# stateless-consensus/phant

Measured on NVIDIA B200. Metric: mpt_proofs_verified_per_sec, higher is better.
Workload: dtype u64

## Files before the change

### phant_b200/csrc/abi.cu

```cuda
#include "../../include/phant_gpu.h"
#include "common.cuh"
#include "ctx.cuh"

#include <cub/device/device_scan.cuh>

#include <stdio.h>
#include <stdlib.h>
#include <string.h>
#include <new>

using namespace phant;

#define CU(expr)                                                              \
    do {                                                                      \
        cudaError_t e_ = (expr);                                              \
        if (e_ != cudaSuccess) return ctx->fail(e_, #expr, __FILE__, __LINE__); \
    } while (0)

int phant_gpu_ctx::fail(cudaError_t e, const char* what, const char* file, int line)
{
    snprintf(last_error, sizeof last_error, "%s: %s (%s:%d)", cudaGetErrorName(e), what, file, line);
    cudaGetLastError();
    return e == cudaErrorMemoryAllocation ? PHANT_GPU_E_OOM : PHANT_GPU_E_CUDA;
}

int DevBuf::reserve(phant_gpu_ctx* ctx, size_t bytes)
{
    if (bytes <= cap) return 0;
    if (ptr) { cudaFree(ptr); ptr = nullptr; cap = 0; }
    size_t want = bytes + bytes / 8 + 256;
    cudaError_t e = cudaMalloc(&ptr, want);
    if (e != cudaSuccess) { want = bytes + 256; e = cudaMalloc(&ptr, want); }
    if (e != cudaSuccess) { ptr = nullptr; return ctx->fail(e, "cudaMalloc", __FILE__, __LINE__); }
    cudaMemsetAsync(ptr, 0, want, ctx->stream);
    cap = want;
    return 0;
}
void DevBuf::release()
{
    if (ptr) cudaFree(ptr);
    ptr = nullptr;
    cap = 0;
}

void phant_gpu_ctx::time_begin(int which)
{
    if ((size_t)n_pairs >= pairs.size()) pairs.emplace_back();
    EventPair& p = pairs[n_pairs];
    if (!p.a) { cudaEventCreate(&p.a); cudaEventCreate(&p.b); }
    p.which = which;
    cudaEventRecord(p.a, stream);
}
void phant_gpu_ctx::time_end()
{
    cudaEventRecord(pairs[n_pairs].b, stream);
    ++n_pairs;
}
void phant_gpu_ctx::resolve_times()
{
    if (!n_pairs) return;
    cudaStreamSynchronize(stream);
    for (int i = 0; i < n_pairs; ++i) {
        float ms = 0.f;
        if (cudaEventElapsedTime(&ms, pairs[i].a, pairs[i].b) == cudaSuccess) {
            if (pairs[i].which == 0) stats.keccak_ms += ms; else stats.walk_ms += ms;
        }
    }
    n_pairs = 0;
}

extern "C" int phant_gpu_abi_version(void) { return PHANT_GPU_ABI_VERSION; }

extern "C" const char* phant_gpu_strerror(int code)
{
    switch (code) {
    case PHANT_GPU_OK: return "ok";
    case PHANT_GPU_E_INVALID: return "invalid argument";
    case PHANT_GPU_E_NO_DEVICE: return "no usable CUDA device";
    case PHANT_GPU_E_OOM: return "out of device memory";
    case PHANT_GPU_E_CUDA: return "CUDA runtime error";
    case PHANT_GPU_E_COMM: return "collective communication error";
    case PHANT_GPU_E_MALFORMED: return "malformed RLP in builder input";
    default: return "unknown error";
    }
}

extern "C" int phant_gpu_create(phant_gpu_ctx** out, const phant_gpu_config* cfg)
{
    if (!out) return PHANT_GPU_E_INVALID;
    *out = nullptr;
    int count = 0;
    if (cudaGetDeviceCount(&count) != cudaSuccess || count == 0) { cudaGetLastError(); return PHANT_GPU_E_NO_DEVICE; }
    int dev = cfg ? cfg->device : 0;
    uint32_t env_flags = 0;
    if (const char* e = getenv("PHANT_GPU_DEVICE")) { char* end = nullptr; const long v = strtol(e, &end, 10); if (end != e && *end == 0) dev = (int)v; }
    if (const char* e = getenv("PHANT_GPU_FLAGS")) { char* end = nullptr; const unsigned long v = strtoul(e, &end, 0); if (end != e && *end == 0) env_flags = (uint32_t)v; }
    if (dev < 0 || dev >= count) return PHANT_GPU_E_INVALID;
    if (cudaSetDevice(dev) != cudaSuccess) { cudaGetLastError(); return PHANT_GPU_E_NO_DEVICE; }
    cudaDeviceProp prop;
    if (cudaGetDeviceProperties(&prop, dev) != cudaSuccess) { cudaGetLastError(); return PHANT_GPU_E_NO_DEVICE; }
    if (prop.major < 10) return PHANT_GPU_E_NO_DEVICE;
    phant_gpu_ctx* ctx = new (std::nothrow) phant_gpu_ctx();
    if (!ctx) return PHANT_GPU_E_OOM;
    ctx->device = dev;
    ctx->flags = (cfg ? cfg->flags : 0) | env_flags;
    if (cudaStreamCreateWithFlags(&ctx->own_stream, cudaStreamNonBlocking) != cudaSuccess) {
        cudaGetLastError();
        delete ctx;
        return PHANT_GPU_E_CUDA;
    }
    ctx->stream = ctx->own_stream;
    if (cudaStreamCreateWithFlags(&ctx->copy_stream, cudaStreamNonBlocking) != cudaSuccess) {
        cudaGetLastError();
        cudaStreamDestroy(ctx->own_stream);
        delete ctx;
        return PHANT_GPU_E_CUDA;
    }
    *out = ctx;
    return PHANT_GPU_OK;
}

extern "C" void phant_gpu_destroy(phant_gpu_ctx* ctx)
{
    if (!ctx) return;
    cudaSetDevice(ctx->device);
    cudaStreamSynchronize(ctx->stream);
    phant_gpu_comm_destroy(ctx);
    for (DevBuf* b : ctx->all_bufs()) b->release();
    for (EventPair& p : ctx->pairs)
        if (p.a) { cudaEventDestroy(p.a); cudaEventDestroy(p.b); }
    for (cudaEvent_t e : ctx->chunk_events) cudaEventDestroy(e);
    if (ctx->copy_stream) cudaStreamDestroy(ctx->copy_stream);
    cudaStreamDestroy(ctx->own_stream);
    delete ctx;
}

extern "C" int phant_gpu_set_flags(phant_gpu_ctx* ctx, uint32_t flags)
{
    if (!ctx) return PHANT_GPU_E_INVALID;
    ctx->flags = flags;
    return PHANT_GPU_OK;
}
extern "C" int phant_gpu_set_stream(phant_gpu_ctx* ctx, void* cuda_stream)
{
    if (!ctx) return PHANT_GPU_E_INVALID;
    ctx->resolve_times();
    ctx->stream = cuda_stream ? (cudaStream_t)cuda_stream : ctx->own_stream;
    return PHANT_GPU_OK;
}
extern "C" const char* phant_gpu_last_error(const phant_gpu_ctx* ctx) { return ctx ? ctx->last_error : "null context"; }

extern "C" int phant_gpu_synchronize(phant_gpu_ctx* ctx)
{
    if (!ctx) return PHANT_GPU_E_INVALID;
    CU(cudaSetDevice(ctx->device));
    CU(cudaStreamSynchronize(ctx->stream));
    if (ctx->comm_stream) CU(cudaStreamSynchronize(ctx->comm_stream));
    return PHANT_GPU_OK;
}
extern "C" int phant_gpu_get_stats(phant_gpu_ctx* ctx, phant_gpu_stats* out)
{
    if (!ctx || !out) return PHANT_GPU_E_INVALID;
    CU(cudaSetDevice(ctx->device));
    ctx->resolve_times();
    CU(cudaStreamSynchronize(ctx->stream));
    if (ctx->perms_pending) {
        unsigned long long p = 0;
        CU(cudaMemcpy(&p, ctx->d_perms.ptr, sizeof p, cudaMemcpyDeviceToHost));
        ctx->stats.keccak_perms += p;
        CU(cudaMemset(ctx->d_perms.ptr, 0, sizeof p));
        ctx->perms_pending = false;
    }
    *out = ctx->stats;
    return PHANT_GPU_OK;
}
extern "C" int phant_gpu_reset_stats(phant_gpu_ctx* ctx)
{
    if (!ctx) return PHANT_GPU_E_INVALID;
    phant_gpu_stats tmp;
    int rc = phant_gpu_get_stats(ctx, &tmp);
    memset(&ctx->stats, 0, sizeof ctx->stats);
    return rc;
}

int phant_gpu_ctx::hash_csr(const uint8_t* d_msgs, const uint64_t* d_off, uint64_t n, uint64_t total_bytes, uint8_t* d_out,
                            uint32_t* d_summary)
{
    phant_gpu_ctx* ctx = this;
    if (n == 0) return PHANT_GPU_OK;
    if (n > 0xffffffffull) return PHANT_GPU_E_INVALID;
    NvtxRange nvtx("phant:keccak");
    KeccakVariant variant = KECCAK_STAGED;
    if (flags & PHANT_GPU_FLAG_KECCAK_DIRECT) variant = KECCAK_DIRECT;
    if (flags & PHANT_GPU_FLAG_KECCAK_WARP) variant = KECCAK_WARP;
    if (variant == KECCAK_STAGED && ((uintptr_t)d_msgs & 15)) variant = KECCAK_DIRECT;

    if (int rc = d_perms.reserve(ctx, 64)) return rc;
    if (!perms_init) { CU(cudaMemsetAsync(d_perms.ptr, 0, 64, stream)); perms_init = true; }
    if (int rc = d_idx.reserve(ctx, keccak_regroup_scratch_bytes(device, n))) return rc;
    CU(launch_keccak_classify(stream, device, d_off, n, (uint32_t*)d_idx.ptr, (uint32_t*)((unsigned long long*)d_perms.ptr + 1),
                              (unsigned long long*)d_perms.ptr));
    stats.launches++;
    perms_pending = true;
    const uint32_t* order = nullptr;
    const bool regroup = !(flags & PHANT_GPU_FLAG_NO_BINNING) && variant != KECCAK_WARP && n >= 4096;
    if (regroup) {
        if (int rc = d_order.reserve(ctx, 4 * n)) return rc;
        CU(launch_keccak_regroup(stream, device, d_off, n, (const uint32_t*)d_idx.ptr, (uint32_t*)d_order.ptr));
        stats.launches++;
        order = (const uint32_t*)d_order.ptr;
    }
    time_begin(0);
    CU(launch_keccak(stream, device, variant, d_msgs, d_off, order, n, d_out, d_summary));
    time_end();
    stats.launches++;
    stats.keccak_msgs += n;
    stats.keccak_bytes += total_bytes;
    return PHANT_GPU_OK;
}

int phant_gpu_ctx::hash_slots(const uint8_t* d_msgs, const uint64_t* d_off, const uint64_t* d_len, uint64_t n, uint8_t* d_out)
{
    phant_gpu_ctx* ctx = this;
    if (n == 0) return PHANT_GPU_OK;
    KeccakVariant variant = KECCAK_STAGED;
    if (flags & PHANT_GPU_FLAG_KECCAK_DIRECT) variant = KECCAK_DIRECT;
    if (flags & PHANT_GPU_FLAG_KECCAK_WARP) variant = KECCAK_WARP;
    if (variant == KECCAK_STAGED && ((uintptr_t)d_msgs & 15)) variant = KECCAK_DIRECT;
    time_begin(0);
    CU(launch_keccak(stream, device, variant, d_msgs, d_off, nullptr, n, d_out, nullptr, d_len));
    time_end();
    stats.launches++;
    stats.keccak_msgs += n;
    return PHANT_GPU_OK;
}

static int check_offsets_host(const uint64_t* off, uint64_t n, uint64_t* total)
{
    for (uint64_t i = 0; i < n; ++i)
        if (off[i + 1] < off[i]) return PHANT_GPU_E_INVALID;
    *total = off[n];
    return PHANT_GPU_OK;
}

extern "C" int phant_gpu_keccak256_batch(phant_gpu_ctx* ctx, const uint8_t* msgs, const uint64_t* off, uint64_t n, uint8_t* out)
{
    if (!ctx || (n && (!off || !out))) return PHANT_GPU_E_INVALID;
    if (n == 0) return PHANT_GPU_OK;
    CU(cudaSetDevice(ctx->device));
    if (ctx->flags & PHANT_GPU_FLAG_DEVICE_PTRS) {
        uint64_t last = 0;
        CU(cudaMemcpyAsync(&last, off + n, 8, cudaMemcpyDeviceToHost, ctx->stream));
        CU(cudaStreamSynchronize(ctx->stream));
        if (last && !msgs) return PHANT_GPU_E_INVALID;
        return ctx->hash_csr(msgs, off, n, last, out);
    }
    uint64_t total = 0;
    if (int rc = check_offsets_host(off, n, &total)) return rc;
    if (total && !msgs) return PHANT_GPU_E_INVALID;
    if (int rc = ctx->d_msgs.reserve(ctx, total + 64)) return rc;
    if (int rc = ctx->d_off.reserve(ctx, 8 * (n + 1))) return rc;
    if (int rc = ctx->d_out.reserve(ctx, 32 * n)) return rc;
    if (total) CU(cudaMemcpyAsync(ctx->d_msgs.ptr, msgs, total, cudaMemcpyHostToDevice, ctx->stream));
    CU(cudaMemcpyAsync(ctx->d_off.ptr, off, 8 * (n + 1), cudaMemcpyHostToDevice, ctx->stream));
    ctx->stats.h2d_bytes += total + 8 * (n + 1);
    if (int rc = ctx->hash_csr((const uint8_t*)ctx->d_msgs.ptr, (const uint64_t*)ctx->d_off.ptr, n, total, (uint8_t*)ctx->d_out.ptr)) return rc;
    CU(cudaMemcpyAsync(out, ctx->d_out.ptr, 32 * n, cudaMemcpyDeviceToHost, ctx->stream));
    ctx->stats.d2h_bytes += 32 * n;
    CU(cudaStreamSynchronize(ctx->stream));
    return PHANT_GPU_OK;
}

extern "C" int phant_gpu_keccak256_batch_async(phant_gpu_ctx* ctx, const uint8_t* msgs, const uint64_t* off, uint64_t n, uint64_t total_bytes,
                                               uint8_t* out)
{
    if (!ctx || (n && (!off || !out)) || (total_bytes && !msgs)) return PHANT_GPU_E_INVALID;
    if (!(ctx->flags & PHANT_GPU_FLAG_DEVICE_PTRS)) return PHANT_GPU_E_INVALID;
    if (n == 0) return PHANT_GPU_OK;
    CU(cudaSetDevice(ctx->device));
    return ctx->hash_csr(msgs, off, n, total_bytes, out);
}

static int verify_dedup_host(phant_gpu_ctx* ctx, const phant_gpu_proof_batch* in, uint64_t* accept_bitmap, uint8_t* status,
                             uint64_t* val_off, uint32_t* val_len)
{
    const uint64_t np = in->n_proofs, n_nodes = in->n_nodes;
    if (n_nodes == 0) return PHANT_GPU_E_INVALID;
    uint64_t total = 0;
    if (int rc = check_offsets_host(in->node_off, n_nodes, &total)) return rc;
    if (total && !in->nodes) return PHANT_GPU_E_INVALID;
    for (uint64_t p = 0; p < np; ++p)
        if (in->proof_first[p + 1] < in->proof_first[p]) return PHANT_GPU_E_INVALID;
    const uint64_t n_refs = in->proof_first[np];
    for (uint64_t r = 0; r < n_refs; ++r)
        if (in->node_index[r] >= n_nodes) return PHANT_GPU_E_INVALID;
    const size_t bm_bytes = ((np + 63) / 64) * 8;
    if (int rc = ctx->d_msgs.reserve(ctx, total + 64)) return rc;
    if (int rc = ctx->d_off.reserve(ctx, 8 * (n_nodes + 1))) return rc;
    if (int rc = ctx->d_first.reserve(ctx, 8 * (np + 1))) return rc;
    if (int rc = ctx->d_index.reserve(ctx, 8 * (n_refs + 1))) return rc;
    if (int rc = ctx->d_keys.reserve(ctx, 32 * np)) return rc;
    if (int rc = ctx->d_roots.reserve(ctx, 32 * in->n_roots)) return rc;
    if (int rc = ctx->d_digests.reserve(ctx, 32 * n_nodes + 32)) return rc;
    if (int rc = ctx->d_summary.reserve(ctx, 4 * n_nodes + 32)) return rc;
    if (int rc = ctx->d_bitmap.reserve(ctx, bm_bytes)) return rc;
    if (int rc = ctx->d_status.reserve(ctx, np)) return rc;
    if (val_off) if (int rc = ctx->d_voff.reserve(ctx, 8 * np)) return rc;
    if (val_len) if (int rc = ctx->d_vlen.reserve(ctx, 4 * np)) return rc;
    cudaStream_t s = ctx->stream;
    if (total) CU(cudaMemcpyAsync(ctx->d_msgs.ptr, in->nodes, total, cudaMemcpyHostToDevice, s));
    CU(cudaMemcpyAsync(ctx->d_off.ptr, in->node_off, 8 * (n_nodes + 1), cudaMemcpyHostToDevice, s));
    CU(cudaMemcpyAsync(ctx->d_first.ptr, in->proof_first, 8 * (np + 1), cudaMemcpyHostToDevice, s));
    if (n_refs) CU(cudaMemcpyAsync(ctx->d_index.ptr, in->node_index, 8 * n_refs, cudaMemcpyHostToDevice, s));
    CU(cudaMemcpyAsync(ctx->d_keys.ptr, in->keys32, 32 * np, cudaMemcpyHostToDevice, s));
    CU(cudaMemcpyAsync(ctx->d_roots.ptr, in->roots32, 32 * in->n_roots, cudaMemcpyHostToDevice, s));
    ctx->stats.h2d_bytes += total + 8 * (n_nodes + 1) + 8 * (np + 1) + 8 * n_refs + 32 * np + 32 * in->n_roots;
    if (int rc = ctx->hash_csr((const uint8_t*)ctx->d_msgs.ptr, (const uint64_t*)ctx->d_off.ptr, n_nodes, total, (uint8_t*)ctx->d_digests.ptr,
                               (uint32_t*)ctx->d_summary.ptr)) return rc;
    CU(cudaMemsetAsync(ctx->d_bitmap.ptr, 0, bm_bytes, s));
    ctx->time_begin(1);
    CU(launch_walk(s, ctx->device, np, (const uint8_t*)ctx->d_msgs.ptr, (const uint64_t*)ctx->d_off.ptr, (const uint64_t*)ctx->d_index.ptr,
                   (const uint64_t*)ctx->d_first.ptr, (const uint8_t*)ctx->d_keys.ptr, (const uint8_t*)ctx->d_roots.ptr, in->n_roots,
                   (const uint8_t*)ctx->d_digests.ptr, (const uint32_t*)ctx->d_summary.ptr, (uint64_t*)ctx->d_bitmap.ptr,
                   (uint8_t*)ctx->d_status.ptr, val_off ? (uint64_t*)ctx->d_voff.ptr : nullptr, val_len ? (uint32_t*)ctx->d_vlen.ptr : nullptr));
    ctx->time_end();
    ctx->stats.launches++;
    if (accept_bitmap) { CU(cudaMemcpyAsync(accept_bitmap, ctx->d_bitmap.ptr, bm_bytes, cudaMemcpyDeviceToHost, s)); ctx->stats.d2h_bytes += bm_bytes; }
    if (status) { CU(cudaMemcpyAsync(status, ctx->d_status.ptr, np, cudaMemcpyDeviceToHost, s)); ctx->stats.d2h_bytes += np; }
    if (val_off) { CU(cudaMemcpyAsync(val_off, ctx->d_voff.ptr, 8 * np, cudaMemcpyDeviceToHost, s)); ctx->stats.d2h_bytes += 8 * np; }
    if (val_len) { CU(cudaMemcpyAsync(val_len, ctx->d_vlen.ptr, 4 * np, cudaMemcpyDeviceToHost, s)); ctx->stats.d2h_bytes += 4 * np; }
    CU(cudaStreamSynchronize(s));
    return PHANT_GPU_OK;
}

extern "C" int phant_gpu_verify_proofs(phant_gpu_ctx* ctx, const phant_gpu_proof_batch* in, uint64_t* accept_bitmap,
                                       uint8_t* status, uint64_t* val_off, uint32_t* val_len)
{
    if (!ctx || !in) return PHANT_GPU_E_INVALID;
    const uint64_t np = in->n_proofs;
    if (np == 0) return PHANT_GPU_OK;
    if (!in->node_off || !in->proof_first || !in->keys32 || !in->roots32) return PHANT_GPU_E_INVALID;
    if (in->n_roots != 1 && in->n_roots != np) return PHANT_GPU_E_INVALID;
    CU(cudaSetDevice(ctx->device));
    const size_t bm_bytes = ((np + 63) / 64) * 8;

    if (ctx->flags & PHANT_GPU_FLAG_DEVICE_PTRS) {
        uint64_t n_nodes = in->n_nodes, total = in->nodes_bytes;
        if (in->node_index && n_nodes == 0) return PHANT_GPU_E_INVALID;
        if (n_nodes == 0) {
            CU(cudaMemcpyAsync(&n_nodes, in->proof_first + np, 8, cudaMemcpyDeviceToHost, ctx->stream));
            CU(cudaStreamSynchronize(ctx->stream));
            if (n_nodes) {
                CU(cudaMemcpyAsync(&total, in->node_off + n_nodes, 8, cudaMemcpyDeviceToHost, ctx->stream));
                CU(cudaStreamSynchronize(ctx->stream));
            }
        }
        if (int rc = ctx->d_digests.reserve(ctx, 32 * n_nodes + 32)) return rc;
        if (int rc = ctx->d_summary.reserve(ctx, 4 * n_nodes + 32)) return rc;
        if (int rc = ctx->hash_csr(in->nodes, in->node_off, n_nodes, total, (uint8_t*)ctx->d_digests.ptr, (uint32_t*)ctx->d_summary.ptr)) return rc;
        NvtxRange nvtx("phant:walk");
        if (int rc = ctx->wait_walk_fence()) return rc;
        if (accept_bitmap) CU(cudaMemsetAsync(accept_bitmap, 0, bm_bytes, ctx->stream));
        ctx->time_begin(1);
        CU(launch_walk(ctx->stream, ctx->device, np, in->nodes, in->node_off, in->node_index, in->proof_first, in->keys32, in->roots32, in->n_roots,
                       (const uint8_t*)ctx->d_digests.ptr, (const uint32_t*)ctx->d_summary.ptr, accept_bitmap, status, val_off, val_len,
                       (const PeerOut*)ctx->walk_peer ));
        ctx->time_end();
        ctx->stats.launches++;
        return PHANT_GPU_OK;
    }

    if (in->node_index) return verify_dedup_host(ctx, in, accept_bitmap, status, val_off, val_len);
    const uint64_t n_nodes = in->proof_first[np];
    const uint64_t total = in->node_off[n_nodes];
    if (total && !in->nodes) return PHANT_GPU_E_INVALID;
    if (int rc = ctx->d_msgs.reserve(ctx, total + 64)) return rc;
    if (int rc = ctx->d_off.reserve(ctx, 8 * (n_nodes + 1))) return rc;
    if (int rc = ctx->d_first.reserve(ctx, 8 * (np + 1))) return rc;
    if (int rc = ctx->d_keys.reserve(ctx, 32 * np)) return rc;
    if (int rc = ctx->d_roots.reserve(ctx, 32 * in->n_roots)) return rc;
    if (int rc = ctx->d_digests.reserve(ctx, 32 * n_nodes + 32)) return rc;
    if (int rc = ctx->d_summary.reserve(ctx, 4 * n_nodes + 32)) return rc;
    if (int rc = ctx->d_bitmap.reserve(ctx, bm_bytes)) return rc;
    if (int rc = ctx->d_status.reserve(ctx, np)) return rc;
    if (val_off) if (int rc = ctx->d_voff.reserve(ctx, 8 * np)) return rc;
    if (val_len) if (int rc = ctx->d_vlen.reserve(ctx, 4 * np)) return rc;
    cudaStream_t s = ctx->stream, cs = ctx->copy_stream;
    uint8_t* d_nodes = (uint8_t*)ctx->d_msgs.ptr;
    uint64_t* d_noff = (uint64_t*)ctx->d_off.ptr;
    uint64_t* d_pfirst = (uint64_t*)ctx->d_first.ptr;
    CU(cudaMemsetAsync(ctx->d_bitmap.ptr, 0, bm_bytes, s));
    CU(cudaMemcpyAsync(ctx->d_roots.ptr, in->roots32, 32 * in->n_roots, cudaMemcpyHostToDevice, s));
    ctx->stats.h2d_bytes += total + 8 * (n_nodes + 1) + 8 * (np + 1) + 32 * np + 32 * in->n_roots;
    static uint64_t chunk_mb = 0;
    if (!chunk_mb) { const char* e = getenv("PHANT_GPU_CHUNK_MB"); const long v = e ? atol(e) : 0; chunk_mb = v >= 1 && v <= 4096 ? (uint64_t)v : 128; }
    const uint64_t target_bytes = chunk_mb << 20;
    uint64_t p0 = 0;
    size_t chunk = 0;
    if (ctx->chunk_events.empty()) { cudaEvent_t e; CU(cudaEventCreateWithFlags(&e, cudaEventDisableTiming)); ctx->chunk_events.push_back(e); }
    CU(cudaEventRecord(ctx->chunk_events[0], s));
    CU(cudaStreamWaitEvent(cs, ctx->chunk_events[0], 0));
    while (p0 < np) {
        uint64_t p1 = p0;
        const uint64_t n0 = in->proof_first[p0], b0 = n0 <= n_nodes ? in->node_off[n0] : 0;
        bool in_range = n0 <= n_nodes;
        do {
            p1 = p1 + 4096 < np ? p1 + 4096 : np;
            in_range = in_range && in->proof_first[p1] <= n_nodes;
        } while (in_range && p1 < np && in->node_off[in->proof_first[p1]] - b0 < target_bytes);
        if (!in_range) {
            cudaStreamSynchronize(cs);
            cudaStreamSynchronize(s);
            return PHANT_GPU_E_INVALID;
        }
        const uint64_t n1 = in->proof_first[p1], b1 = in->node_off[n1];
        {
            bool ok = n0 <= n1 && n1 <= n_nodes && b0 <= b1 && b1 <= total;
            for (uint64_t p = p0; ok && p < p1; ++p) ok = in->proof_first[p] <= in->proof_first[p + 1];
            for (uint64_t j = n0; ok && j < n1; ++j) ok = in->node_off[j] <= in->node_off[j + 1];
            if (!ok) {
                cudaStreamSynchronize(cs);
                cudaStreamSynchronize(s);
                return PHANT_GPU_E_INVALID;
            }
        }
        nvtxRangePushA("phant:h2d chunk");
        if (b1 > b0) CU(cudaMemcpyAsync(d_nodes + b0, in->nodes + b0, b1 - b0, cudaMemcpyHostToDevice, cs));
        CU(cudaMemcpyAsync(d_noff + n0, in->node_off + n0, 8 * (n1 - n0 + 1), cudaMemcpyHostToDevice, cs));
        CU(cudaMemcpyAsync(d_pfirst + p0, in->proof_first + p0, 8 * (p1 - p0 + 1), cudaMemcpyHostToDevice, cs));
        CU(cudaMemcpyAsync((uint8_t*)ctx->d_keys.ptr + 32 * p0, in->keys32 + 32 * p0, 32 * (p1 - p0), cudaMemcpyHostToDevice, cs));
        ++chunk;
        if (ctx->chunk_events.size() <= chunk) { cudaEvent_t e; CU(cudaEventCreateWithFlags(&e, cudaEventDisableTiming)); ctx->chunk_events.push_back(e); }
        CU(cudaEventRecord(ctx->chunk_events[chunk], cs));
        CU(cudaStreamWaitEvent(s, ctx->chunk_events[chunk], 0));
        nvtxRangePop();
        if (int rc = ctx->hash_csr(d_nodes, d_noff + n0, n1 - n0, b1 - b0, (uint8_t*)ctx->d_digests.ptr + 32 * n0,
                                   (uint32_t*)ctx->d_summary.ptr + n0)) {
            cudaStreamSynchronize(cs);
            cudaStreamSynchronize(s);
            return rc;
        }
        ctx->time_begin(1);
        CU(launch_walk(s, ctx->device, p1 - p0, d_nodes, d_noff, nullptr, d_pfirst + p0, (const uint8_t*)ctx->d_keys.ptr + 32 * p0,
                       (const uint8_t*)ctx->d_roots.ptr + (in->n_roots == 1 ? 0 : 32 * p0), in->n_roots, (const uint8_t*)ctx->d_digests.ptr,
                       (const uint32_t*)ctx->d_summary.ptr, (uint64_t*)ctx->d_bitmap.ptr + p0 / 64, (uint8_t*)ctx->d_status.ptr + p0, val_off ? (uint64_t*)ctx->d_voff.ptr + p0 : nullptr,
                       val_len ? (uint32_t*)ctx->d_vlen.ptr + p0 : nullptr));
        ctx->time_end();
        ctx->stats.launches++;
        p0 = p1;
    }
    if (accept_bitmap) { CU(cudaMemcpyAsync(accept_bitmap, ctx->d_bitmap.ptr, bm_bytes, cudaMemcpyDeviceToHost, s)); ctx->stats.d2h_bytes += bm_bytes; }
    if (status) { CU(cudaMemcpyAsync(status, ctx->d_status.ptr, np, cudaMemcpyDeviceToHost, s)); ctx->stats.d2h_bytes += np; }
    if (val_off) { CU(cudaMemcpyAsync(val_off, ctx->d_voff.ptr, 8 * np, cudaMemcpyDeviceToHost, s)); ctx->stats.d2h_bytes += 8 * np; }
    if (val_len) { CU(cudaMemcpyAsync(val_len, ctx->d_vlen.ptr, 4 * np, cudaMemcpyDeviceToHost, s)); ctx->stats.d2h_bytes += 4 * np; }
    CU(cudaStreamSynchronize(s));
    return PHANT_GPU_OK;
}

extern "C" int phant_gpu_verify_witness(phant_gpu_ctx* ctx, const phant_gpu_witness* in, uint64_t* accept_bitmap, uint8_t* status,
                                        uint64_t* val_off, uint32_t* val_len)
{
    if (!ctx || !in) return PHANT_GPU_E_INVALID;
    const uint64_t nk = in->n_keys, nn = in->n_nodes;
    if (nk == 0) return PHANT_GPU_OK;
    if (!in->keys32 || !in->roots32 || (nn && !in->node_off) || (in->n_roots != 1 && in->n_roots != nk)) return PHANT_GPU_E_INVALID;
    if (nn > (1ull << 30)) return PHANT_GPU_E_INVALID;
    CU(cudaSetDevice(ctx->device));
    cudaStream_t s = ctx->stream;
    const bool dev = ctx->flags & PHANT_GPU_FLAG_DEVICE_PTRS;
    const size_t bm_bytes = ((nk + 63) / 64) * 8;
    uint64_t total = in->nodes_bytes;
    const uint8_t* d_nodes = in->nodes; const uint64_t* d_noff = in->node_off; const uint8_t* d_keys = in->keys32; const uint8_t* d_roots = in->roots32;
    uint64_t* d_bitmap = accept_bitmap; uint8_t* d_status = status; uint64_t* d_voff = val_off; uint32_t* d_vlen = val_len;
    if (!dev) {
        total = 0;
        if (nn) { if (int rc = check_offsets_host(in->node_off, nn, &total)) return rc; }
        if (total && !in->nodes) return PHANT_GPU_E_INVALID;
        if (int rc = ctx->d_msgs.reserve(ctx, total + 64)) return rc;
        if (int rc = ctx->d_off.reserve(ctx, 8 * (nn + 1))) return rc;
        if (int rc = ctx->d_keys.reserve(ctx, 32 * nk)) return rc;
        if (int rc = ctx->d_roots.reserve(ctx, 32 * in->n_roots)) return rc;
        if (int rc = ctx->d_bitmap.reserve(ctx, bm_bytes)) return rc;
        if (int rc = ctx->d_status.reserve(ctx, nk)) return rc;
        if (val_off) if (int rc = ctx->d_voff.reserve(ctx, 8 * nk)) return rc;
        if (val_len) if (int rc = ctx->d_vlen.reserve(ctx, 4 * nk)) return rc;
        if (total) CU(cudaMemcpyAsync(ctx->d_msgs.ptr, in->nodes, total, cudaMemcpyHostToDevice, s));
        static const uint64_t zero2[2] = {0, 0};
        CU(cudaMemcpyAsync(ctx->d_off.ptr, nn ? in->node_off : zero2, 8 * (nn + 1), cudaMemcpyHostToDevice, s));
        CU(cudaMemcpyAsync(ctx->d_keys.ptr, in->keys32, 32 * nk, cudaMemcpyHostToDevice, s));
        CU(cudaMemcpyAsync(ctx->d_roots.ptr, in->roots32, 32 * in->n_roots, cudaMemcpyHostToDevice, s));
        ctx->stats.h2d_bytes += total + 8 * (nn + 1) + 32 * nk + 32 * in->n_roots;
        d_nodes = (const uint8_t*)ctx->d_msgs.ptr; d_noff = (const uint64_t*)ctx->d_off.ptr; d_keys = (const uint8_t*)ctx->d_keys.ptr;
        d_roots = (const uint8_t*)ctx->d_roots.ptr; d_bitmap = (uint64_t*)ctx->d_bitmap.ptr; d_status = (uint8_t*)ctx->d_status.ptr;
        d_voff = val_off ? (uint64_t*)ctx->d_voff.ptr : nullptr; d_vlen = val_len ? (uint32_t*)ctx->d_vlen.ptr : nullptr;
    }
    uint32_t capacity = 64;
    while ((uint64_t)capacity < 2 * nn) capacity <<= 1;
    if (int rc = ctx->d_digests.reserve(ctx, 32 * nn + 32)) return rc;
    if (int rc = ctx->d_summary.reserve(ctx, 4 * nn + 32)) return rc;
    if (int rc = ctx->d_index.reserve(ctx, 4ull * capacity)) return rc;
    if (int rc = ctx->hash_csr(d_nodes, d_noff, nn, total, (uint8_t*)ctx->d_digests.ptr, (uint32_t*)ctx->d_summary.ptr)) return rc;
    CU(launch_bag_build(s, ctx->device, (const uint8_t*)ctx->d_digests.ptr, nn, (uint32_t*)ctx->d_index.ptr, capacity));
    if (d_bitmap) CU(cudaMemsetAsync(d_bitmap, 0, bm_bytes, s));
    ctx->time_begin(1);
    CU(launch_walk_bag(s, ctx->device, nk, d_nodes, d_noff, d_keys, d_roots, in->n_roots, (const uint8_t*)ctx->d_digests.ptr,
                       (const uint32_t*)ctx->d_summary.ptr, (const uint32_t*)ctx->d_index.ptr, capacity, d_bitmap, d_status, d_voff, d_vlen));
    ctx->time_end();
    ctx->stats.launches += 2;
    if (!dev) {
        if (accept_bitmap) { CU(cudaMemcpyAsync(accept_bitmap, d_bitmap, bm_bytes, cudaMemcpyDeviceToHost, s)); ctx->stats.d2h_bytes += bm_bytes; }
        if (status) { CU(cudaMemcpyAsync(status, d_status, nk, cudaMemcpyDeviceToHost, s)); ctx->stats.d2h_bytes += nk; }
        if (val_off) { CU(cudaMemcpyAsync(val_off, d_voff, 8 * nk, cudaMemcpyDeviceToHost, s)); ctx->stats.d2h_bytes += 8 * nk; }
        if (val_len) { CU(cudaMemcpyAsync(val_len, d_vlen, 4 * nk, cudaMemcpyDeviceToHost, s)); ctx->stats.d2h_bytes += 4 * nk; }
        CU(cudaStreamSynchronize(s));
    }
    return PHANT_GPU_OK;
}

__global__ void bloom_set_kernel(const uint8_t* __restrict__ digests, const uint32_t* __restrict__ bloom_of_item, uint64_t n_items,
                                 uint64_t n_blooms, uint32_t* __restrict__ blooms )
{
    for (uint64_t i = (uint64_t)blockIdx.x * blockDim.x + threadIdx.x; i < n_items; i += (uint64_t)gridDim.x * blockDim.x) {
        const uint64_t b = bloom_of_item[i];
        if (b >= n_blooms) continue;
        const uint8_t* h = digests + 32 * i;
#pragma unroll
        for (int j = 0; j < 3; ++j) {
            const uint32_t bit_to_set = (((uint32_t)h[2 * j] << 8) | h[2 * j + 1]) & 0x07ffu;
            const uint32_t bit_index = 0x07ffu - bit_to_set;
            const uint32_t byte_index = bit_index >> 3;
            const uint32_t in_byte = 1u << (7 - (bit_index & 7));
            atomicOr(&blooms[64 * b + (byte_index >> 2)], in_byte << (8 * (byte_index & 3)));
        }
    }
}

extern "C" int phant_gpu_logs_bloom(phant_gpu_ctx* ctx, const uint8_t* items, const uint64_t* item_off, const uint32_t* bloom_of_item,
                                    uint64_t n_items, uint64_t n_blooms, uint8_t* blooms)
{
    if (!ctx || (n_blooms && !blooms) || (n_items && (!item_off || !bloom_of_item))) return PHANT_GPU_E_INVALID;
    if (n_blooms == 0) return n_items ? PHANT_GPU_E_INVALID : PHANT_GPU_OK;
    CU(cudaSetDevice(ctx->device));
    cudaStream_t s = ctx->stream;
    const bool dev = ctx->flags & PHANT_GPU_FLAG_DEVICE_PTRS;
    const uint8_t* d_items = items; const uint64_t* d_ioff = item_off; const uint32_t* d_map = bloom_of_item;
    uint32_t* d_blooms = (uint32_t*)blooms;
    uint64_t total = 0;
    if (!dev) {
        if (n_items) {
            if (int rc = check_offsets_host(item_off, n_items, &total)) return rc;
            if (total && !items) return PHANT_GPU_E_INVALID;
            for (uint64_t i = 0; i < n_items; ++i) if (bloom_of_item[i] >= n_blooms) return PHANT_GPU_E_INVALID;
        }
        if (int rc = ctx->d_msgs.reserve(ctx, total + 64)) return rc;
        if (int rc = ctx->d_off.reserve(ctx, 8 * (n_items + 1))) return rc;
        if (int rc = ctx->d_index.reserve(ctx, 4 * (n_items + 1))) return rc;
        if (int rc = ctx->d_out.reserve(ctx, 256 * n_blooms)) return rc;
        if (total) CU(cudaMemcpyAsync(ctx->d_msgs.ptr, items, total, cudaMemcpyHostToDevice, s));
        if (n_items) {
            CU(cudaMemcpyAsync(ctx->d_off.ptr, item_off, 8 * (n_items + 1), cudaMemcpyHostToDevice, s));
            CU(cudaMemcpyAsync(ctx->d_index.ptr, bloom_of_item, 4 * n_items, cudaMemcpyHostToDevice, s));
        }
        ctx->stats.h2d_bytes += total + 12 * n_items + 8;
        d_items = (const uint8_t*)ctx->d_msgs.ptr; d_ioff = (const uint64_t*)ctx->d_off.ptr; d_map = (const uint32_t*)ctx->d_index.ptr;
        d_blooms = (uint32_t*)ctx->d_out.ptr;
    } else if (n_items) {
        CU(cudaMemcpyAsync(&total, item_off + n_items, 8, cudaMemcpyDeviceToHost, s));
        CU(cudaStreamSynchronize(s));
    }
    CU(cudaMemsetAsync(d_blooms, 0, 256 * n_blooms, s));
    if (n_items) {
        if (int rc = ctx->d_digests.reserve(ctx, 32 * n_items + 32)) return rc;
        if (int rc = ctx->hash_csr(d_items, d_ioff, n_items, total, (uint8_t*)ctx->d_digests.ptr)) return rc;
        uint64_t blocks = (n_items + 255) / 256;
        const uint64_t cap = (uint64_t)keccak_num_sms(ctx->device) * 8;
        if (blocks > cap) blocks = cap;
        bloom_set_kernel<<<(unsigned)blocks, 256, 0, s>>>((const uint8_t*)ctx->d_digests.ptr, d_map, n_items, n_blooms, d_blooms);
        CU(cudaGetLastError());
        ctx->stats.launches++;
    }
    if (!dev) {
        CU(cudaMemcpyAsync(blooms, d_blooms, 256 * n_blooms, cudaMemcpyDeviceToHost, s));
        ctx->stats.d2h_bytes += 256 * n_blooms;
        CU(cudaStreamSynchronize(s));
    }
    return PHANT_GPU_OK;
}

namespace phant { uint64_t synth_c2_bytes_per_proof(uint32_t depth); }

static int c3_scans(phant_gpu_ctx* ctx, uint64_t seed, uint64_t first_index, uint64_t n)
{
    if (int rc = ctx->d_tmp_a.reserve(ctx, 8 * (n + 1))) return rc;
    if (int rc = ctx->d_tmp_b.reserve(ctx, 8 * (n + 1))) return rc;
    if (int rc = ctx->d_scan_a.reserve(ctx, 8 * (n + 1))) return rc;
    if (int rc = ctx->d_scan_b.reserve(ctx, 8 * (n + 1))) return rc;
    CU(cudaMemsetAsync((uint64_t*)ctx->d_tmp_a.ptr + n, 0, 8, ctx->stream));
    CU(cudaMemsetAsync((uint64_t*)ctx->d_tmp_b.ptr + n, 0, 8, ctx->stream));
    CU(launch_synth_c3_sizes(ctx->stream, ctx->device, seed, first_index, n, (uint64_t*)ctx->d_tmp_a.ptr, (uint64_t*)ctx->d_tmp_b.ptr));
    ctx->stats.launches++;
    size_t temp = 0;
    CU(cub::DeviceScan::ExclusiveSum(nullptr, temp, (const uint64_t*)ctx->d_tmp_a.ptr, (uint64_t*)ctx->d_scan_a.ptr, (int64_t)(n + 1), ctx->stream));
    if (int rc = ctx->d_cub.reserve(ctx, temp)) return rc;
    CU(cub::DeviceScan::ExclusiveSum(ctx->d_cub.ptr, temp, (const uint64_t*)ctx->d_tmp_a.ptr, (uint64_t*)ctx->d_scan_a.ptr, (int64_t)(n + 1), ctx->stream));
    CU(cub::DeviceScan::ExclusiveSum(ctx->d_cub.ptr, temp, (const uint64_t*)ctx->d_tmp_b.ptr, (uint64_t*)ctx->d_scan_b.ptr, (int64_t)(n + 1), ctx->stream));
    return PHANT_GPU_OK;
}

extern "C" int phant_gpu_synth_sizes(phant_gpu_ctx* ctx, int which, uint64_t seed, uint64_t first_index, uint64_t n, uint32_t depth,
                                     uint64_t* total_nodes, uint64_t* total_bytes)
{
    if (!ctx || !total_nodes || !total_bytes) return PHANT_GPU_E_INVALID;
    CU(cudaSetDevice(ctx->device));
    if (which == 2) {
        if (depth < 2 || depth > 64) return PHANT_GPU_E_INVALID;
        *total_nodes = n * depth;
        *total_bytes = n * synth_c2_bytes_per_proof(depth);
        return PHANT_GPU_OK;
    }
    if (which != 3) return PHANT_GPU_E_INVALID;
    *total_nodes = *total_bytes = 0;
    if (n == 0) return PHANT_GPU_OK;
    if (int rc = c3_scans(ctx, seed, first_index, n)) return rc;
    CU(cudaMemcpyAsync(total_nodes, (uint64_t*)ctx->d_scan_a.ptr + n, 8, cudaMemcpyDeviceToHost, ctx->stream));
    CU(cudaMemcpyAsync(total_bytes, (uint64_t*)ctx->d_scan_b.ptr + n, 8, cudaMemcpyDeviceToHost, ctx->stream));
    CU(cudaStreamSynchronize(ctx->stream));
    return PHANT_GPU_OK;
}

extern "C" int phant_gpu_synth(phant_gpu_ctx* ctx, int which, uint64_t seed, uint64_t first_index, uint64_t n, uint32_t depth,
                               int corrupt, uint8_t* nodes, uint64_t* node_off, uint64_t* proof_first, uint8_t* keys32, uint8_t* roots32)
{
    if (!ctx || !nodes || !node_off || !proof_first || !keys32 || !roots32) return PHANT_GPU_E_INVALID;
    if (n == 0) return PHANT_GPU_OK;
    CU(cudaSetDevice(ctx->device));
    if (which == 2) {
        if (depth < 2 || depth > 64) return PHANT_GPU_E_INVALID;
        CU(launch_synth_c2(ctx->stream, ctx->device, seed, first_index, n, depth, corrupt, nodes, node_off, proof_first, keys32, roots32));
        ctx->stats.launches++;
    } else if (which == 3) {
        if (int rc = c3_scans(ctx, seed, first_index, n)) return rc;
        CU(cudaMemcpyAsync(proof_first, ctx->d_scan_a.ptr, 8 * (n + 1), cudaMemcpyDeviceToDevice, ctx->stream));
        CU(launch_synth_c3(ctx->stream, ctx->device, seed, first_index, n, corrupt, (const uint64_t*)ctx->d_scan_a.ptr,
                           (const uint64_t*)ctx->d_scan_b.ptr, nodes, node_off, keys32, roots32));
        ctx->stats.launches++;
    } else {
        return PHANT_GPU_E_INVALID;
    }
    CU(cudaStreamSynchronize(ctx->stream));
    return PHANT_GPU_OK;
}
```

### phant_b200/csrc/common.cuh

```cuda
#pragma once
#include <cuda_runtime.h>
#include <stdint.h>

namespace phant {

enum KeccakVariant { KECCAK_STAGED = 0, KECCAK_DIRECT = 1, KECCAK_WARP = 2 };

int keccak_num_sms(int device);
cudaError_t launch_keccak(cudaStream_t s, int device, KeccakVariant variant, const uint8_t* msgs, const uint64_t* off,
                          const uint32_t* order, uint64_t n, uint8_t* out, uint32_t* summary ,
                          const uint64_t* len = nullptr );
uint64_t keccak_regroup_scratch_bytes(int device, uint64_t n);
cudaError_t launch_keccak_classify(cudaStream_t s, int device, const uint64_t* off, uint64_t n, uint32_t* hist, uint32_t* ticket,
                                   unsigned long long* perms);
cudaError_t launch_keccak_regroup(cudaStream_t s, int device, const uint64_t* off, uint64_t n, const uint32_t* start, uint32_t* order);

constexpr int PEER_MAX_WORLD = 16;
struct PeerOut {
    uint32_t* dst[PEER_MAX_WORLD];
    unsigned long long* ready[PEER_MAX_WORLD];
    const unsigned long long* done;
    unsigned long long wait_done;
    unsigned long long step;
    uint32_t* ticket;
    uint32_t* err;
    uint32_t world;
};

cudaError_t launch_walk(cudaStream_t s, int device, uint64_t n_proofs, const uint8_t* nodes, const uint64_t* node_off,
                        const uint64_t* node_index , const uint64_t* proof_first, const uint8_t* keys32, const uint8_t* roots32, uint64_t n_roots,
                        const uint8_t* digests, const uint32_t* summary , uint64_t* bitmap, uint8_t* status,
                        uint64_t* val_off, uint32_t* val_len, const PeerOut* peer = nullptr );

cudaError_t launch_peer_collect(cudaStream_t s, const unsigned long long* ready, uint32_t world, unsigned long long step, const void* src, void* dst,
                                uint64_t bytes, const PeerOut& sig);

cudaError_t launch_bag_build(cudaStream_t s, int device, const uint8_t* digests, uint64_t n_nodes, uint32_t* table, uint32_t capacity);
cudaError_t launch_walk_bag(cudaStream_t s, int device, uint64_t n_keys, const uint8_t* nodes, const uint64_t* node_off, const uint8_t* keys32,
                            const uint8_t* roots32, uint64_t n_roots, const uint8_t* digests, const uint32_t* summary, const uint32_t* table,
                            uint32_t capacity, uint64_t* bitmap, uint8_t* status, uint64_t* val_off, uint32_t* val_len);

cudaError_t launch_synth_c2(cudaStream_t s, int device, uint64_t seed, uint64_t first_index, uint64_t n, uint32_t depth,
                            int corrupt, uint8_t* nodes, uint64_t* node_off, uint64_t* proof_first, uint8_t* keys32,
                            uint8_t* roots32);
cudaError_t launch_synth_c3_sizes(cudaStream_t s, int device, uint64_t seed, uint64_t first_index, uint64_t n,
                                  uint64_t* n_nodes_per, uint64_t* n_bytes_per);
cudaError_t launch_synth_c3(cudaStream_t s, int device, uint64_t seed, uint64_t first_index, uint64_t n, int corrupt,
                            const uint64_t* node_first ,
                            const uint64_t* byte_first , uint8_t* nodes,
                            uint64_t* node_off, uint8_t* keys32, uint8_t* roots32);

}
```

### phant_b200/csrc/keccak_f1600.cuh

```cuda
#pragma once
#include <stdint.h>

namespace phant {

__constant__ uint64_t KECCAK_RC[24] = {
    0x0000000000000001ull, 0x0000000000008082ull, 0x800000000000808aull, 0x8000000080008000ull,
    0x000000000000808bull, 0x0000000080000001ull, 0x8000000080008081ull, 0x8000000000008009ull,
    0x000000000000008aull, 0x0000000000000088ull, 0x0000000080008009ull, 0x000000008000000aull,
    0x000000008000808bull, 0x800000000000008bull, 0x8000000000008089ull, 0x8000000000008003ull,
    0x8000000000008002ull, 0x8000000000000080ull, 0x000000000000800aull, 0x800000008000000aull,
    0x8000000080008081ull, 0x8000000000008080ull, 0x0000000080000001ull, 0x8000000080008008ull};

constexpr int KECCAK_RATE = 136;
constexpr int KECCAK_RATE_WORDS = 17;

template <int N>
__device__ __forceinline__ uint64_t rol64(uint64_t x)
{
    if constexpr (N == 0) return x;
    const uint32_t lo = (uint32_t)x, hi = (uint32_t)(x >> 32);
    uint32_t rlo, rhi;
    if constexpr (N == 32) {
        rlo = hi; rhi = lo;
    } else if constexpr (N < 32) {
        rlo = __funnelshift_l(hi, lo, N);
        rhi = __funnelshift_l(lo, hi, N);
    } else {
        rlo = __funnelshift_l(lo, hi, N - 32);
        rhi = __funnelshift_l(hi, lo, N - 32);
    }
    return ((uint64_t)rhi << 32) | rlo;
}

#define PHANT_RHOPI(I, J, R) b[J] = rol64<R>(a[I] ^ c[((I) % 5 + 4) % 5] ^ r1[((I) % 5 + 1) % 5]);

__device__ __forceinline__ void keccak_round(uint64_t (&a)[25], uint64_t rc)
{
    uint64_t c[5], r1[5], b[25];
#pragma unroll
    for (int x = 0; x < 5; ++x) c[x] = a[x] ^ a[x + 5] ^ a[x + 10] ^ a[x + 15] ^ a[x + 20];
#pragma unroll
    for (int x = 0; x < 5; ++x) r1[x] = rol64<1>(c[x]);
    PHANT_RHOPI(0, 0, 0)    PHANT_RHOPI(1, 10, 1)   PHANT_RHOPI(2, 20, 62)  PHANT_RHOPI(3, 5, 28)   PHANT_RHOPI(4, 15, 27)
    PHANT_RHOPI(5, 16, 36)  PHANT_RHOPI(6, 1, 44)   PHANT_RHOPI(7, 11, 6)   PHANT_RHOPI(8, 21, 55)  PHANT_RHOPI(9, 6, 20)
    PHANT_RHOPI(10, 7, 3)   PHANT_RHOPI(11, 17, 10) PHANT_RHOPI(12, 2, 43)  PHANT_RHOPI(13, 12, 25) PHANT_RHOPI(14, 22, 39)
    PHANT_RHOPI(15, 23, 41) PHANT_RHOPI(16, 8, 45)  PHANT_RHOPI(17, 18, 15) PHANT_RHOPI(18, 3, 21)  PHANT_RHOPI(19, 13, 8)
    PHANT_RHOPI(20, 14, 18) PHANT_RHOPI(21, 24, 2)  PHANT_RHOPI(22, 9, 61)  PHANT_RHOPI(23, 19, 56) PHANT_RHOPI(24, 4, 14)
#pragma unroll
    for (int y = 0; y < 25; y += 5) {
#pragma unroll
        for (int x = 0; x < 5; ++x) a[y + x] = b[y + x] ^ (~b[y + (x + 1) % 5] & b[y + (x + 2) % 5]);
    }
    a[0] ^= rc;
}

__device__ __forceinline__ void keccak_last_round_digest(uint64_t (&a)[25], uint64_t rc)
{
    uint64_t c[5], r1[5], b[5];
#pragma unroll
    for (int x = 0; x < 5; ++x) c[x] = a[x] ^ a[x + 5] ^ a[x + 10] ^ a[x + 15] ^ a[x + 20];
#pragma unroll
    for (int x = 0; x < 5; ++x) r1[x] = rol64<1>(c[x]);
    PHANT_RHOPI(0, 0, 0) PHANT_RHOPI(6, 1, 44) PHANT_RHOPI(12, 2, 43) PHANT_RHOPI(18, 3, 21) PHANT_RHOPI(24, 4, 14)
#pragma unroll
    for (int x = 0; x < 4; ++x) a[x] = b[x] ^ (~b[(x + 1) % 5] & b[(x + 2) % 5]);
    a[0] ^= rc;
}
#undef PHANT_RHOPI

template <int UNROLL = 2, bool DIGEST_ONLY = false>
__device__ __forceinline__ void keccak_f1600(uint64_t (&a)[25])
{
    constexpr int LOOPED = DIGEST_ONLY ? 24 - UNROLL : 24;
#pragma unroll 1
    for (int r = 0; r < LOOPED; r += UNROLL) {
#pragma unroll
        for (int k = 0; k < UNROLL; ++k) keccak_round(a, KECCAK_RC[r + k]);
    }
    if constexpr (DIGEST_ONLY) {
#pragma unroll
        for (int k = 0; k < UNROLL - 1; ++k) keccak_round(a, KECCAK_RC[LOOPED + k]);
        keccak_last_round_digest(a, KECCAK_RC[23]);
    }
}

struct MsgView {
    const uint64_t* w;
    uint32_t sh;
};
__device__ __forceinline__ MsgView msg_view(const void* p)
{
    const uintptr_t a = (uintptr_t)p;
    return MsgView{(const uint64_t*)(a & ~(uintptr_t)7), (uint32_t)(a & 7) * 8};
}
__device__ __forceinline__ uint64_t funnel64(uint64_t lo, uint64_t hi, uint32_t sh)
{
    return sh ? (lo >> sh) | (hi << (64 - sh)) : lo;
}

template <int UNROLL>
__device__ __forceinline__ void absorb_full(uint64_t (&st)[25], const MsgView& v, uint32_t base)
{
    uint64_t w[KECCAK_RATE_WORDS + 1];
#pragma unroll
    for (int k = 0; k < KECCAK_RATE_WORDS; ++k) w[k] = v.w[base + k];
    w[KECCAK_RATE_WORDS] = v.sh ? v.w[base + KECCAK_RATE_WORDS] : 0;
#pragma unroll
    for (int k = 0; k < KECCAK_RATE_WORDS; ++k) st[k] ^= funnel64(w[k], w[k + 1], v.sh);
    keccak_f1600<UNROLL>(st);
}

template <int UNROLL>
__device__ __forceinline__ void absorb_final(uint64_t (&st)[25], const MsgView& v, uint32_t base, uint32_t rem)
{
    const uint32_t mis = v.sh >> 3;
#pragma unroll
    for (int k = 0; k < KECCAK_RATE_WORDS; ++k) {
        const int valid = (int)rem - 8 * k;
        uint64_t word = 0;
        if (valid > 0) {
            const uint64_t lo = v.w[base + k];
            const uint64_t hi = (mis + (valid > 8 ? 8 : valid) > 8) ? v.w[base + k + 1] : 0;
            word = funnel64(lo, hi, v.sh);
            if (valid < 8) word &= (1ull << (8 * valid)) - 1;
        }
        if (valid >= 0 && valid < 8) word ^= 1ull << (8 * valid);
        st[k] ^= word;
    }
    st[KECCAK_RATE_WORDS - 1] ^= 0x8000000000000000ull;
    keccak_f1600<UNROLL, true>(st);
}

#ifndef PHANT_HOST_SMEM
__device__ __forceinline__ uint32_t lds32(uint32_t saddr)
{
    uint32_t v;
    asm volatile("ld.shared.u32 %0, [%1];" : "=r"(v) : "r"(saddr));
    return v;
}
#else
__device__ __forceinline__ uint32_t lds32(uint32_t saddr) { uint32_t v; memcpy(&v, PHANT_HOST_SMEM + saddr, 4); return v; }
#endif
template <int UNROLL, bool DIGEST_ONLY = false>
__device__ __forceinline__ void absorb_full_smem(uint64_t (&st)[25], uint32_t sa)
{
    const uint32_t a4 = sa & ~3u, sh = (sa & 3u) * 8;
    uint32_t w[2 * KECCAK_RATE_WORDS + 1];
#pragma unroll
    for (int j = 0; j < 2 * KECCAK_RATE_WORDS; ++j) w[j] = lds32(a4 + 4 * j);
    w[2 * KECCAK_RATE_WORDS] = sh ? lds32(a4 + 4 * 2 * KECCAK_RATE_WORDS) : 0;
#pragma unroll
    for (int k = 0; k < KECCAK_RATE_WORDS; ++k) {
        const uint32_t lo = __funnelshift_r(w[2 * k], w[2 * k + 1], sh);
        const uint32_t hi = __funnelshift_r(w[2 * k + 1], w[2 * k + 2], sh);
        st[k] ^= ((uint64_t)hi << 32) | lo;
    }
    keccak_f1600<UNROLL, DIGEST_ONLY>(st);
}
#ifndef PHANT_HOST_SMEM
__device__ __forceinline__ void sts32_(uint32_t saddr, uint32_t v) { asm volatile("st.shared.u32 [%0], %1;" ::"r"(saddr), "r"(v) : "memory"); }
#else
__device__ __forceinline__ void sts32_(uint32_t saddr, uint32_t v) { memcpy(PHANT_HOST_SMEM + saddr, &v, 4); }
#endif
template <int UNROLL>
__device__ __forceinline__ void absorb_final_smem_masked(uint64_t (&st)[25], uint32_t sa, uint32_t rem)
{
    const uint32_t a4 = sa & ~3u, sh = (sa & 3u) * 8;
    const uint32_t nfw = rem >> 2, tail = rem & 3u;
    const uint32_t bmask = (1u << (8 * tail)) - 1u, pad = 1u << (8 * tail);
    uint32_t prev = rem ? lds32(a4) : 0;
#pragma unroll
    for (int j = 0; j < 2 * KECCAK_RATE_WORDS; ++j) {
        uint32_t word = 0;
        if ((uint32_t)j < nfw || ((uint32_t)j == nfw && tail)) {
            const uint32_t next = lds32(a4 + 4 * (j + 1));
            word = __funnelshift_r(prev, next, sh);
            prev = next;
        }
        if ((uint32_t)j == nfw) word = (word & bmask) ^ pad;
        if (j == 2 * KECCAK_RATE_WORDS - 1) word ^= 0x80000000u;
        st[j >> 1] ^= (j & 1) ? ((uint64_t)word << 32) : (uint64_t)word;
    }
    keccak_f1600<UNROLL, true>(st);
}
template <int UNROLL>
__device__ __forceinline__ void absorb_final_smem(uint64_t (&st)[25], uint32_t sa, uint32_t rem, uint32_t room)
{
    if (room < KECCAK_RATE + 4) { absorb_final_smem_masked<UNROLL>(st, sa, rem); return; }
    const uint32_t a4 = sa & ~3u, s = sa & 3u;
    const uint32_t p0 = rem + s, p1 = KECCAK_RATE - 1 + s;
    const uint32_t q0 = p0 >> 2, b0 = p0 & 3u, q1 = p1 >> 2, b1 = p1 & 3u;
    uint32_t w0 = lds32(a4 + 4 * q0);
    w0 = (w0 & ((1u << (8 * b0)) - 1u)) | (1u << (8 * b0));
    if (q0 == q1) w0 |= 0x80u << (8 * b1);
    sts32_(a4 + 4 * q0, w0);
    for (uint32_t q = q0 + 1; q < q1; ++q) sts32_(a4 + 4 * q, 0u);
    if (q1 > q0) sts32_(a4 + 4 * q1, 0x80u << (8 * b1));
    absorb_full_smem<UNROLL, true>(st, sa);
}

template <int UNROLL = 2>
__device__ __forceinline__ void keccak256_thread(const uint8_t* p, uint64_t len, uint64_t (&digest)[4])
{
    uint64_t st[25];
#pragma unroll
    for (int i = 0; i < 25; ++i) st[i] = 0;
    const MsgView v = msg_view(p);
    uint32_t base = 0;
    while (len >= KECCAK_RATE) {
        absorb_full<UNROLL>(st, v, base);
        base += KECCAK_RATE_WORDS;
        len -= KECCAK_RATE;
    }
    absorb_final<UNROLL>(st, v, base, (uint32_t)len);
#pragma unroll
    for (int i = 0; i < 4; ++i) digest[i] = st[i];
}

}
```

### phant_b200/csrc/keccak_kernels.cu

```cuda
#include "common.cuh"
#include "keccak_f1600.cuh"
#include "node_summary.cuh"

#include <stdlib.h>
#include <string.h>

namespace phant {

template <int UNROLL>
__global__ void __launch_bounds__(128)
keccak256_direct_kernel(const uint8_t* __restrict__ msgs, const uint64_t* __restrict__ off,
                        const uint32_t* __restrict__ order, uint64_t n, uint8_t* __restrict__ out,
                        uint32_t* __restrict__ summary, const uint64_t* __restrict__ len)
{
    for (uint64_t i = (uint64_t)blockIdx.x * blockDim.x + threadIdx.x; i < n; i += (uint64_t)gridDim.x * blockDim.x) {
        const uint64_t m = order ? order[i] : i;
        const uint64_t beg = off[m], end = len ? beg + len[m] : off[m + 1];
        uint64_t dg[4];
        keccak256_thread<UNROLL>(msgs + beg, end - beg, dg);
        if (summary) summary[m] = (end - beg) <= 4096 ? summarize_node(msgs + beg, (uint32_t)(end - beg)) : 0;
        uint64_t* o = reinterpret_cast<uint64_t*>(out + 32 * m);
        o[0] = dg[0]; o[1] = dg[1]; o[2] = dg[2]; o[3] = dg[3];
    }
}

constexpr int stage_window(int blocks)
{
    int s = (blocks * KECCAK_RATE + 15 + 15) / 16;
    if (s % 2 == 0) ++s;
    return 16 * s;
}
constexpr int stage_slot(int blocks) { return stage_window(blocks) + 32; }
constexpr int stage_smem(int blocks, int warps) { return 128 + warps * 32 * stage_slot(blocks) + 16; }
static_assert(stage_smem(4, 12) <= 232448, "default shape must fit the 227 KB a CTA may opt into");

__device__ __forceinline__ uint32_t smem_u32(const void* p) { return (uint32_t)__cvta_generic_to_shared(p); }
__device__ __forceinline__ void mbar_init(uint32_t bar, uint32_t count)
{
    asm volatile("mbarrier.init.shared::cta.b64 [%0], %1;" ::"r"(bar), "r"(count));
}
__device__ __forceinline__ void mbar_arrive(uint32_t bar)
{
    asm volatile("mbarrier.arrive.shared::cta.b64 _, [%0];" ::"r"(bar) : "memory");
}
__device__ __forceinline__ void mbar_arrive_expect_tx(uint32_t bar, uint32_t bytes)
{
    asm volatile("mbarrier.arrive.expect_tx.shared::cta.b64 _, [%0], %1;" ::"r"(bar), "r"(bytes) : "memory");
}
__device__ __forceinline__ void mbar_wait(uint32_t bar, uint32_t parity)
{
    asm volatile(
        "{\n"
        ".reg .pred P1;\n"
        "LAB_WAIT:\n"
        "mbarrier.try_wait.parity.shared::cta.b64 P1, [%0], %1;\n"
        "@P1 bra DONE;\n"
        "bra LAB_WAIT;\n"
        "DONE:\n"
        "}" ::"r"(bar), "r"(parity) : "memory");
}
__device__ __forceinline__ void bulk_g2s(uint32_t dst, const void* src, uint32_t bytes, uint32_t bar)
{
    asm volatile("cp.async.bulk.shared::cluster.global.mbarrier::complete_tx::bytes [%0], [%1], %2, [%3];"
                 ::"r"(dst), "l"(src), "r"(bytes), "r"(bar) : "memory");
}
__device__ __forceinline__ void fence_proxy_async() { asm volatile("fence.proxy.async.shared::cta;" ::: "memory"); }

template <int UNROLL, int BLOCKS, int WARPS>
__global__ void __launch_bounds__(WARPS * 32)
keccak256_staged_kernel(const uint8_t* __restrict__ msgs, const uint64_t* __restrict__ off,
                        const uint32_t* __restrict__ order, uint64_t n, uint8_t* __restrict__ out,
                        uint32_t* __restrict__ summary, const uint64_t* __restrict__ len)
{
    extern __shared__ __align__(128) uint8_t smem[];
    const uint32_t warp = threadIdx.x >> 5, lane = threadIdx.x & 31;
    const uint32_t bar = smem_u32(smem) + 8 * warp;
    constexpr int SLOT = stage_slot(BLOCKS), WINDOW = stage_window(BLOCKS);
    uint8_t* slot = smem + 128 + (warp * 32 + lane) * SLOT;
    const uint32_t slot_s = smem_u32(slot);
    if (lane == 0) mbar_init(bar, 32);
    fence_proxy_async();
    __syncthreads();
    uint32_t parity = 0;

    const uint64_t n_tiles = (n + 31) / 32;
    for (uint64_t tile = (uint64_t)blockIdx.x * WARPS + warp; tile < n_tiles; tile += (uint64_t)gridDim.x * WARPS) {
        const uint64_t idx = tile * 32 + lane;
        const bool active = idx < n;
        uint64_t m = 0, cur = 0, end = 0;
        if (active) {
            m = order ? order[idx] : idx;
            cur = off[m];
            end = len ? cur + len[m] : off[m + 1];
        }
        uint64_t st[25];
#pragma unroll
        for (int i = 0; i < 25; ++i) st[i] = 0;
        bool done = !active;
        bool first_trip = true;

        while (!__all_sync(0xffffffffu, done)) {
            const uint64_t need = done ? 0 : end - cur;
            const uint64_t a0 = cur & ~(uint64_t)15;
            uint32_t cs = 0;
            if (need) {
                const uint64_t span = ((end - a0) + 15) & ~(uint64_t)15;
                cs = span < WINDOW ? (uint32_t)span : WINDOW;
                fence_proxy_async();
                mbar_arrive_expect_tx(bar, cs);
                bulk_g2s(slot_s, msgs + a0, cs, bar);
            } else {
                mbar_arrive(bar);
            }
            mbar_wait(bar, parity);
            parity ^= 1;
            if (!done) {
                const uint32_t skew = (uint32_t)(cur - a0);
                const uint64_t in_slot = cs - skew;
                const uint64_t avail = need < in_slot ? need : in_slot;
                if (summary && first_trip)
                    summary[m] = avail == need ? summarize_node(slot + skew, (uint32_t)need) : 0;
                const uint32_t nfull = (uint32_t)(avail / KECCAK_RATE);
                uint32_t sa = slot_s + skew;
                for (uint32_t b = 0; b < nfull; ++b) {
                    absorb_full_smem<UNROLL>(st, sa);
                    sa += KECCAK_RATE;
                }
                if (avail == need) {
                    absorb_final_smem<UNROLL>(st, sa, (uint32_t)(avail - (uint64_t)nfull * KECCAK_RATE), slot_s + SLOT - sa);
                    done = true;
                } else {
                    cur += (uint64_t)nfull * KECCAK_RATE;
                }
            }
            first_trip = false;
        }
        if (active) {
            uint4* o = reinterpret_cast<uint4*>(out + 32 * m);
            o[0] = make_uint4((uint32_t)st[0], (uint32_t)(st[0] >> 32), (uint32_t)st[1], (uint32_t)(st[1] >> 32));
            o[1] = make_uint4((uint32_t)st[2], (uint32_t)(st[2] >> 32), (uint32_t)st[3], (uint32_t)(st[3] >> 32));
        }
    }
}

__device__ __forceinline__ uint64_t rolv64(uint64_t x, uint32_t n) { return n ? (x << n) | (x >> (64 - n)) : x; }

__global__ void __launch_bounds__(256)
keccak256_warp_kernel(const uint8_t* __restrict__ msgs, const uint64_t* __restrict__ off, uint64_t n,
                      uint8_t* __restrict__ out, const uint64_t* __restrict__ lens)
{
    const uint32_t lane = threadIdx.x & 31;
    const uint64_t warp_id = ((uint64_t)blockIdx.x * blockDim.x + threadIdx.x) >> 5;
    const uint64_t n_warps = ((uint64_t)gridDim.x * blockDim.x) >> 5;
    const uint32_t x = lane % 5, y = (lane % 25) / 5;
    constexpr uint32_t RHO[25] = {0, 1, 62, 28, 27, 36, 44, 6, 55, 20, 3, 10, 43, 25, 39, 41, 45, 15, 21, 8, 18, 2, 61, 56, 14};
    uint32_t rho = 0;
#pragma unroll
    for (int i = 0; i < 25; ++i) if (lane == (uint32_t)i) rho = RHO[i];
    const uint32_t pi_src = ((x + 3 * y) % 5) + 5 * x;
    const uint32_t col1 = (x + 1) % 5, col4 = (x + 4) % 5;
    const uint32_t row1 = 5 * y + (x + 1) % 5, row2 = 5 * y + (x + 2) % 5;
    const uint32_t FULL = 0xffffffffu;

    for (uint64_t m = warp_id; m < n; m += n_warps) {
        const uint64_t beg = off[m], end = lens ? beg + lens[m] : off[m + 1];
        uint64_t len = end - beg;
        const MsgView v = msg_view(msgs + beg);
        uint64_t s = 0;
        uint32_t base = 0;
        bool last = false;
        while (!last) {
            uint64_t word = 0;
            if (len >= KECCAK_RATE) {
                uint64_t lo = 0;
                if (lane <= KECCAK_RATE_WORDS && (lane < KECCAK_RATE_WORDS || v.sh)) lo = v.w[base + lane];
                const uint64_t hi = __shfl_down_sync(FULL, lo, 1);
                word = lane < KECCAK_RATE_WORDS ? funnel64(lo, hi, v.sh) : 0;
                len -= KECCAK_RATE;
                base += KECCAK_RATE_WORDS;
            } else {
                const uint32_t rem = (uint32_t)len, mis = v.sh >> 3;
                const uint32_t n_al = (mis + rem + 7) / 8;
                uint64_t lo = (rem && lane < n_al) ? v.w[base + lane] : 0;
                const uint64_t hi = __shfl_down_sync(FULL, lo, 1);
                if (lane < KECCAK_RATE_WORDS) {
                    const int valid = (int)rem - 8 * (int)lane;
                    if (valid > 0) {
                        word = funnel64(lo, hi, v.sh);
                        if (valid < 8) word &= (1ull << (8 * valid)) - 1;
                    }
                    if (valid >= 0 && valid < 8) word ^= 1ull << (8 * valid);
                    if (lane == KECCAK_RATE_WORDS - 1) word ^= 0x8000000000000000ull;
                }
                last = true;
            }
            s ^= word;
#pragma unroll 1
            for (int r = 0; r < 24; ++r) {
                uint64_t c = s;
                c ^= __shfl_sync(FULL, s, (lane + 5) % 25);
                c ^= __shfl_sync(FULL, s, (lane + 10) % 25);
                c ^= __shfl_sync(FULL, s, (lane + 15) % 25);
                c ^= __shfl_sync(FULL, s, (lane + 20) % 25);
                const uint64_t cm = __shfl_sync(FULL, c, col4), cp = __shfl_sync(FULL, c, col1);
                s ^= cm ^ rolv64(cp, 1);
                s = rolv64(s, rho);
                s = __shfl_sync(FULL, s, pi_src);
                const uint64_t b1 = __shfl_sync(FULL, s, row1), b2 = __shfl_sync(FULL, s, row2);
                s ^= ~b1 & b2;
                if (lane == 0) s ^= KECCAK_RC[r];
            }
        }
        if (lane < 4) reinterpret_cast<uint64_t*>(out + 32 * m)[lane] = s;
    }
}

constexpr int CLS_THREADS = 256, CLS_WARPS = CLS_THREADS / 32;

__device__ __forceinline__ uint32_t keccak_class_of(uint64_t len)
{
    const uint64_t nb = len / KECCAK_RATE + 1;
    return (uint32_t)(15 - (nb > 16 ? 15 : nb - 1));
}

__global__ void __launch_bounds__(CLS_THREADS)
keccak_class_kernel(const uint64_t* __restrict__ off, uint64_t n, uint64_t chunk, uint32_t* __restrict__ hist ,
                    uint32_t* __restrict__ ticket, unsigned long long* __restrict__ perms)
{
    __shared__ uint32_t h[16];
    __shared__ uint32_t cls_total[16];
    __shared__ bool last;
    if (threadIdx.x < 16) h[threadIdx.x] = 0;
    __syncthreads();
    const uint64_t lo = (uint64_t)blockIdx.x * chunk, hi = lo + chunk < n ? lo + chunk : n;
    unsigned long long local = 0;
    for (uint64_t i0 = lo; i0 < hi; i0 += CLS_THREADS) {
        const uint64_t i = i0 + threadIdx.x;
        const bool valid = i < hi;
        uint32_t c = 16;
        if (valid) {
            const uint64_t len = off[i + 1] - off[i];
            c = keccak_class_of(len);
            local += len / KECCAK_RATE + 1;
        }
        const uint32_t peers = __match_any_sync(0xffffffffu, c);
        if (valid && (threadIdx.x & 31) == (uint32_t)(__ffs(peers) - 1)) atomicAdd(&h[c], __popc(peers));
    }
    for (int o = 16; o; o >>= 1) local += __shfl_down_sync(0xffffffffu, local, o);
    if ((threadIdx.x & 31) == 0 && local) atomicAdd(perms, local);
    __syncthreads();
    if (threadIdx.x < 16) hist[16 * blockIdx.x + threadIdx.x] = h[threadIdx.x];
    __threadfence();
    __syncthreads();
    if (threadIdx.x == 0) last = atomicAdd(ticket, 1u) == gridDim.x - 1;
    __syncthreads();
    if (!last) return;
    __threadfence();
    const uint32_t nb = gridDim.x, warp = threadIdx.x >> 5, lane = threadIdx.x & 31;
    for (uint32_t c = warp; c < 16; c += CLS_WARPS) {
        uint32_t t = 0;
        for (uint32_t b = lane; b < nb; b += 32) t += __ldcg(&hist[16 * b + c]);
        for (int o = 16; o; o >>= 1) t += __shfl_down_sync(0xffffffffu, t, o);
        if (lane == 0) cls_total[c] = t;
    }
    __syncthreads();
    for (uint32_t c = warp; c < 16; c += CLS_WARPS) {
        uint32_t carry = 0;
        for (uint32_t k = 0; k < c; ++k) carry += cls_total[k];
        for (uint32_t b0 = 0; b0 < nb; b0 += 32) {
            const uint32_t b = b0 + lane;
            const uint32_t v = b < nb ? __ldcg(&hist[16 * b + c]) : 0;
            uint32_t incl = v;
            for (int o = 1; o < 32; o <<= 1) {
                const uint32_t up = __shfl_up_sync(0xffffffffu, incl, o);
                if (lane >= (uint32_t)o) incl += up;
            }
            if (b < nb) hist[16 * b + c] = carry + incl - v;
            carry += __shfl_sync(0xffffffffu, incl, 31);
        }
    }
    if (threadIdx.x == 0) *ticket = 0;
}

__global__ void __launch_bounds__(CLS_THREADS)
keccak_regroup_kernel(const uint64_t* __restrict__ off, uint64_t n, uint64_t chunk, const uint32_t* __restrict__ start ,
                      uint32_t* __restrict__ order)
{
    __shared__ uint32_t base[16];
    __shared__ uint32_t wcnt[CLS_WARPS][16];
    const uint32_t warp = threadIdx.x >> 5, lane = threadIdx.x & 31;
    if (threadIdx.x < 16) base[threadIdx.x] = start[16 * blockIdx.x + threadIdx.x];
    const uint64_t lo = (uint64_t)blockIdx.x * chunk, hi = lo + chunk < n ? lo + chunk : n;
    for (uint64_t i0 = lo; i0 < hi; i0 += CLS_THREADS) {
        if (threadIdx.x < CLS_WARPS * 16) (&wcnt[0][0])[threadIdx.x] = 0;
        __syncthreads();
        const uint64_t i = i0 + threadIdx.x;
        const bool valid = i < hi;
        const uint32_t c = valid ? keccak_class_of(off[i + 1] - off[i]) : 16;
        const uint32_t peers = __match_any_sync(0xffffffffu, c);
        const uint32_t rank = __popc(peers & ((1u << lane) - 1u));
        if (valid && rank == 0) wcnt[warp][c] = __popc(peers);
        __syncthreads();
        if (valid) {
            uint32_t pos = base[c] + rank;
            for (uint32_t w = 0; w < warp; ++w) pos += wcnt[w][c];
            order[pos] = (uint32_t)i;
        }
        __syncthreads();
        if (threadIdx.x < 16) {
            uint32_t t = 0;
#pragma unroll
            for (int w = 0; w < CLS_WARPS; ++w) t += wcnt[w][threadIdx.x];
            base[threadIdx.x] += t;
        }
        __syncthreads();
    }
}

int keccak_num_sms(int device)
{
    static int cached[64] = {0};
    if (device < 0 || device >= 64) device = 0;
    if (!cached[device]) cudaDeviceGetAttribute(&cached[device], cudaDevAttrMultiProcessorCount, device);
    return cached[device] ? cached[device] : 148;
}

template <int BLOCKS, int WARPS>
static cudaError_t launch_staged(cudaStream_t s, int device, int sms, const uint8_t* msgs, const uint64_t* off, const uint32_t* order, uint64_t n,
                                 uint8_t* out, uint32_t* summary, const uint64_t* len)
{
    constexpr int SMEM = stage_smem(BLOCKS, WARPS);
    static int ctas_cache[64] = {0};
    int& ctas_per_sm = ctas_cache[(device >= 0 && device < 64) ? device : 0];
    if (!ctas_per_sm) {
        cudaError_t e = cudaFuncSetAttribute(keccak256_staged_kernel<2, BLOCKS, WARPS>, cudaFuncAttributeMaxDynamicSharedMemorySize, SMEM);
        if (e != cudaSuccess) return e;
        cudaFuncSetAttribute(keccak256_staged_kernel<2, BLOCKS, WARPS>, cudaFuncAttributePreferredSharedMemoryCarveout, 100);
        e = cudaOccupancyMaxActiveBlocksPerMultiprocessor(&ctas_per_sm, keccak256_staged_kernel<2, BLOCKS, WARPS>, WARPS * 32, SMEM);
        if (e != cudaSuccess || ctas_per_sm < 1) { ctas_per_sm = 0; return e != cudaSuccess ? e : cudaErrorLaunchOutOfResources; }
    }
    const uint64_t tiles = (n + 31) / 32;
    uint64_t blocks = (tiles + WARPS - 1) / WARPS;
    const uint64_t cap = (uint64_t)sms * ctas_per_sm;
    if (blocks > cap) blocks = cap;
    keccak256_staged_kernel<2, BLOCKS, WARPS><<<(unsigned)blocks, WARPS * 32, SMEM, s>>>(msgs, off, order, n, out, summary, len);
    return cudaGetLastError();
}

cudaError_t launch_keccak(cudaStream_t s, int device, KeccakVariant variant, const uint8_t* msgs, const uint64_t* off,
                          const uint32_t* order, uint64_t n, uint8_t* out, uint32_t* summary, const uint64_t* len)
{
    if (n == 0) return cudaSuccess;
    const int sms = keccak_num_sms(device);
    switch (variant) {
    case KECCAK_STAGED: {
        static int cfg = -1;
        if (cfg < 0) {
            const char* e = getenv("PHANT_STAGE_CFG");
            cfg = 0;
            if (e) {
                const char* names[] = {"default", "b3w4", "b2w4", "b1w4", "b4w8", "b2w8", "b4w12", "b4w6", "b3w8", "b4w10", "b4w4"};
                for (int i = 0; i < 11; ++i) if (!strcmp(e, names[i])) cfg = i;
            }
        }
        switch (cfg) {
        case 1: return launch_staged<3, 4>(s, device, sms, msgs, off, order, n, out, summary, len);
        case 2: return launch_staged<2, 4>(s, device, sms, msgs, off, order, n, out, summary, len);
        case 3: return launch_staged<1, 4>(s, device, sms, msgs, off, order, n, out, summary, len);
        case 4: return launch_staged<4, 8>(s, device, sms, msgs, off, order, n, out, summary, len);
        case 5: return launch_staged<2, 8>(s, device, sms, msgs, off, order, n, out, summary, len);
        case 6: return launch_staged<4, 12>(s, device, sms, msgs, off, order, n, out, summary, len);
        case 7: return launch_staged<4, 6>(s, device, sms, msgs, off, order, n, out, summary, len);
        case 8: return launch_staged<3, 8>(s, device, sms, msgs, off, order, n, out, summary, len);
        case 9: return launch_staged<4, 10>(s, device, sms, msgs, off, order, n, out, summary, len);
        case 10: return launch_staged<4, 4>(s, device, sms, msgs, off, order, n, out, summary, len);
        default: return launch_staged<4, 12>(s, device, sms, msgs, off, order, n, out, summary, len);
        }
    }
    case KECCAK_DIRECT: {
        uint64_t blocks = (n + 127) / 128;
        const uint64_t cap = (uint64_t)sms * 8;
        if (blocks > cap) blocks = cap;
        keccak256_direct_kernel<2><<<(unsigned)blocks, 128, 0, s>>>(msgs, off, order, n, out, summary, len);
        break;
    }
    case KECCAK_WARP: {
        uint64_t blocks = (n + 7) / 8;
        const uint64_t cap = (uint64_t)sms * 8;
        if (blocks > cap) blocks = cap;
        keccak256_warp_kernel<<<(unsigned)blocks, 256, 0, s>>>(msgs, off, n, out, len);
        if (summary) cudaMemsetAsync(summary, 0, 4 * n, s);
        break;
    }
    }
    return cudaGetLastError();
}

static void class_geometry(int device, uint64_t n, uint64_t& blocks, uint64_t& chunk)
{
    const uint64_t cap = (uint64_t)keccak_num_sms(device) * 8;
    chunk = ((n + cap - 1) / cap + CLS_THREADS - 1) / CLS_THREADS * CLS_THREADS;
    blocks = (n + chunk - 1) / chunk;
}
uint64_t keccak_regroup_scratch_bytes(int device, uint64_t n)
{
    uint64_t blocks, chunk;
    class_geometry(device, n ? n : 1, blocks, chunk);
    return 64 * blocks;
}
cudaError_t launch_keccak_classify(cudaStream_t s, int device, const uint64_t* off, uint64_t n, uint32_t* hist, uint32_t* ticket,
                                   unsigned long long* perms)
{
    if (n == 0) return cudaSuccess;
    uint64_t blocks, chunk;
    class_geometry(device, n, blocks, chunk);
    keccak_class_kernel<<<(unsigned)blocks, CLS_THREADS, 0, s>>>(off, n, chunk, hist, ticket, perms);
    return cudaGetLastError();
}
cudaError_t launch_keccak_regroup(cudaStream_t s, int device, const uint64_t* off, uint64_t n, const uint32_t* start, uint32_t* order)
{
    if (n == 0) return cudaSuccess;
    uint64_t blocks, chunk;
    class_geometry(device, n, blocks, chunk);
    keccak_regroup_kernel<<<(unsigned)blocks, CLS_THREADS, 0, s>>>(off, n, chunk, start, order);
    return cudaGetLastError();
}

}
```

### phant_b200/csrc/walk_kernel.cu

```cuda
#include "common.cuh"

#include <stdlib.h>

#include "walk_one.cuh"

namespace phant {
namespace {

__device__ __forceinline__ unsigned long long ld_acquire_sys(const unsigned long long* p)
{
    unsigned long long v;
    asm volatile("ld.acquire.sys.global.u64 %0, [%1];" : "=l"(v) : "l"(p) : "memory");
    return v;
}
__device__ __forceinline__ void st_release_sys(unsigned long long* p, unsigned long long v)
{
    asm volatile("st.release.sys.global.u64 [%0], %1;" ::"l"(p), "l"(v) : "memory");
}
__device__ __forceinline__ unsigned long long global_timer_ns()
{
    unsigned long long t;
    asm volatile("mov.u64 %0, %globaltimer;" : "=l"(t));
    return t;
}
__device__ __forceinline__ void wait_flags(const unsigned long long* flags, uint32_t world, unsigned long long value, uint32_t* err)
{
    const unsigned long long t0 = global_timer_ns();
    for (uint32_t r = 0; r < world; ++r)
        while (ld_acquire_sys(flags + r) < value)
            if (global_timer_ns() - t0 > 4000000000ull) { *err = 1; return; }
}

template <bool BAG, int MINB, bool PEER = false>
__global__ void __launch_bounds__(128, MINB)
walk_kernel(const Bag bag, uint64_t n_proofs, const uint8_t* __restrict__ nodes, const uint64_t* __restrict__ node_off,
            const uint64_t* __restrict__ node_index, const uint64_t* __restrict__ proof_first, const uint8_t* __restrict__ keys32,
            const uint8_t* __restrict__ roots32, uint64_t n_roots, const uint8_t* __restrict__ digests,
            const uint32_t* __restrict__ summary, uint64_t* __restrict__ bitmap, uint8_t* __restrict__ status, uint64_t* __restrict__ val_off,
            uint32_t* __restrict__ val_len, const PeerOut peer)
{
    if (PEER) {
        if (threadIdx.x == 0 && peer.wait_done) wait_flags(peer.done, peer.world, peer.wait_done, peer.err);
        __syncthreads();
    }
    const uint64_t n_padded = (n_proofs + 31) & ~(uint64_t)31;
    for (uint64_t p = (uint64_t)blockIdx.x * blockDim.x + threadIdx.x; p < n_padded; p += (uint64_t)gridDim.x * blockDim.x) {
        int st = ST_REJECT;
        if (p < n_proofs) {
            uint64_t vo;
            uint32_t vl;
            st = walk_one<BAG>(nodes, node_off, node_index, bag, BAG ? 0 : proof_first[p], BAG ? 0 : proof_first[p + 1], keys32 + 32 * p,
                          roots32 + (n_roots == 1 ? 0 : 32 * p), digests, summary, vo, vl);
            if (status) status[p] = (uint8_t)st;
            if (val_off) val_off[p] = vo;
            if (val_len) val_len[p] = vl;
        }
        const uint32_t word = __ballot_sync(0xffffffffu, st == ST_PRESENT || st == ST_ABSENT);
        if (PEER) {
            const uint32_t lane = threadIdx.x & 31;
            if (lane < peer.world) peer.dst[lane][p >> 5] = word;
        } else if (bitmap && (threadIdx.x & 31) == 0) reinterpret_cast<uint32_t*>(bitmap)[p >> 5] = word;
    }
    if (PEER) {
        __threadfence_system();
        __syncthreads();
        if (threadIdx.x == 0) {
            const uint32_t t = atomicAdd(peer.ticket, 1u);
            if (t == gridDim.x - 1) {
                __threadfence_system();
                for (uint32_t r = 0; r < peer.world; ++r) st_release_sys(peer.ready[r], peer.step);
                *peer.ticket = 0;
            }
        }
    }
}

}

static int walk_minb()
{
    static int v = -1;
    if (v < 0) {
        const char* e = getenv("PHANT_WALK_MINB");
        v = e ? atoi(e) : 8;
        if (v != 6 && v != 10 && v != 12 && v != 16) v = 8;
    }
    return v;
}

cudaError_t launch_walk(cudaStream_t s, int device, uint64_t n_proofs, const uint8_t* nodes, const uint64_t* node_off,
                        const uint64_t* node_index, const uint64_t* proof_first, const uint8_t* keys32, const uint8_t* roots32, uint64_t n_roots,
                        const uint8_t* digests, const uint32_t* summary, uint64_t* bitmap, uint8_t* status, uint64_t* val_off,
                        uint32_t* val_len, const PeerOut* peer)
{
    if (n_proofs == 0) return cudaSuccess;
    uint64_t blocks = (n_proofs + 127) / 128;
    const uint64_t cap = (uint64_t)keccak_num_sms(device) * 16;
    if (blocks > cap) blocks = cap;
    if (peer) {
        walk_kernel<false, 8, true><<<(unsigned)blocks, 128, 0, s>>>(Bag{nullptr, 0}, n_proofs, nodes, node_off, node_index, proof_first, keys32, roots32, n_roots,
                                                                    digests, summary, bitmap, status, val_off, val_len, *peer);
        return cudaGetLastError();
    }
#define PHANT_WALK_ARGS Bag{nullptr, 0}, n_proofs, nodes, node_off, node_index, proof_first, keys32, roots32, n_roots, digests, summary, bitmap, status, val_off, val_len, PeerOut{}
    switch (walk_minb()) {
    case 6: walk_kernel<false, 6><<<(unsigned)blocks, 128, 0, s>>>(PHANT_WALK_ARGS); break;
    case 10: walk_kernel<false, 10><<<(unsigned)blocks, 128, 0, s>>>(PHANT_WALK_ARGS); break;
    case 12: walk_kernel<false, 12><<<(unsigned)blocks, 128, 0, s>>>(PHANT_WALK_ARGS); break;
    case 16: walk_kernel<false, 16><<<(unsigned)blocks, 128, 0, s>>>(PHANT_WALK_ARGS); break;
    default: walk_kernel<false, 8><<<(unsigned)blocks, 128, 0, s>>>(PHANT_WALK_ARGS); break;
    }
#undef PHANT_WALK_ARGS
    return cudaGetLastError();
}

namespace {
__global__ void bag_insert_kernel(const uint8_t* __restrict__ digests, uint64_t n_nodes, uint32_t* __restrict__ table, uint32_t mask)
{
    for (uint64_t i = (uint64_t)blockIdx.x * blockDim.x + threadIdx.x; i < n_nodes; i += (uint64_t)gridDim.x * blockDim.x) {
        uint32_t e[8];
        load32_aligned(digests + 32 * i, e);
        uint32_t s = bag_slot(e, mask);
        for (;;) {
            const uint32_t prev = atomicCAS(&table[s], BAG_EMPTY, (uint32_t)i);
            if (prev == BAG_EMPTY) break;
            if (eq32_aligned(digests + 32ull * prev, e)) break;
            s = (s + 1) & mask;
        }
    }
}
}

cudaError_t launch_bag_build(cudaStream_t s, int device, const uint8_t* digests, uint64_t n_nodes, uint32_t* table, uint32_t capacity)
{
    cudaError_t e = cudaMemsetAsync(table, 0xff, 4ull * capacity, s);
    if (e != cudaSuccess || n_nodes == 0) return e;
    uint64_t blocks = (n_nodes + 255) / 256;
    const uint64_t cap = (uint64_t)keccak_num_sms(device) * 8;
    if (blocks > cap) blocks = cap;
    bag_insert_kernel<<<(unsigned)blocks, 256, 0, s>>>(digests, n_nodes, table, capacity - 1);
    return cudaGetLastError();
}

cudaError_t launch_walk_bag(cudaStream_t s, int device, uint64_t n_keys, const uint8_t* nodes, const uint64_t* node_off, const uint8_t* keys32,
                            const uint8_t* roots32, uint64_t n_roots, const uint8_t* digests, const uint32_t* summary, const uint32_t* table,
                            uint32_t capacity, uint64_t* bitmap, uint8_t* status, uint64_t* val_off, uint32_t* val_len)
{
    if (n_keys == 0) return cudaSuccess;
    uint64_t blocks = (n_keys + 127) / 128;
    const uint64_t cap = (uint64_t)keccak_num_sms(device) * 16;
    if (blocks > cap) blocks = cap;
    walk_kernel<true, 8><<<(unsigned)blocks, 128, 0, s>>>(Bag{table, capacity - 1}, n_keys, nodes, node_off, nullptr, nullptr, keys32, roots32, n_roots,
                                                      digests, summary, bitmap, status, val_off, val_len, PeerOut{});
    return cudaGetLastError();
}

namespace {
__global__ void __launch_bounds__(256)
peer_collect_kernel(const unsigned long long* __restrict__ ready , uint32_t world, unsigned long long step,
                    const unsigned long long* __restrict__ src, unsigned long long* __restrict__ dst, uint64_t n_words,
                    const PeerOut sig )
{
    if (threadIdx.x == 0) wait_flags(ready, world, step, sig.err);
    __syncthreads();
    for (uint64_t i = (uint64_t)blockIdx.x * blockDim.x + threadIdx.x; i < n_words; i += (uint64_t)gridDim.x * blockDim.x) dst[i] = __ldcv(src + i);
    __threadfence_system();
    __syncthreads();
    if (threadIdx.x == 0) {
        const uint32_t t = atomicAdd(sig.ticket, 1u);
        if (t == gridDim.x - 1) {
            __threadfence_system();
            for (uint32_t r = 0; r < world; ++r) st_release_sys(sig.ready[r], step);
            *sig.ticket = 0;
        }
    }
}
}

cudaError_t launch_peer_collect(cudaStream_t s, const unsigned long long* ready, uint32_t world, unsigned long long step, const void* src, void* dst,
                                uint64_t bytes, const PeerOut& sig)
{
    const uint64_t n_words = bytes / 8;
    uint64_t blocks = (n_words + 255) / 256;
    if (blocks > 64) blocks = 64;
    if (blocks == 0) blocks = 1;
    peer_collect_kernel<<<(unsigned)blocks, 256, 0, s>>>(ready, world, step, (const unsigned long long*)src, (unsigned long long*)dst, n_words, sig);
    return cudaGetLastError();
}

}
```

### phant_b200/csrc/walk_one.cuh

```cuda
#pragma once
#include <stdint.h>

namespace phant {
namespace {

enum { ST_REJECT = 0, ST_PRESENT = 1, ST_ABSENT = 2, ST_MISSING = 3 };

constexpr uint32_t BAG_EMPTY = 0xffffffffu;
struct Bag {
    const uint32_t* table;
    uint32_t mask;
};

struct Item {
    uint32_t is_list;
    uint32_t pay_off;
    uint32_t pay_len;
};

__device__ __forceinline__ uint32_t rlp_item(const uint8_t* p, uint32_t avail, Item& it)
{
    if (avail == 0) return 0;
    const uint32_t b = p[0];
    if (b < 0x80) { it.is_list = 0; it.pay_off = 0; it.pay_len = 1; return 1; }
    const uint32_t is_list = b >= 0xc0;
    const uint32_t base_short = is_list ? 0xc0 : 0x80, base_long = is_list ? 0xf7 : 0xb7;
    it.is_list = is_list;
    if (b <= base_long) {
        const uint32_t len = b - base_short;
        if (1 + len > avail) return 0;
        if (!is_list && len == 1 && p[1] < 0x80) return 0;
        it.pay_off = 1; it.pay_len = len;
        return 1 + len;
    }
    const uint32_t n = b - base_long;
    if (n > 4 || 1 + n > avail) return 0;
    if (p[1] == 0) return 0;
    uint64_t len = 0;
    for (uint32_t i = 0; i < n; ++i) len = (len << 8) | p[1 + i];
    if (len <= 55) return 0;
    if (1 + n + len > avail) return 0;
    it.pay_off = 1 + n; it.pay_len = (uint32_t)len;
    return (uint32_t)(1 + n + len);
}

__device__ __forceinline__ void load32_aligned(const uint8_t* a, uint32_t (&e)[8])
{
    const uint4 lo = __ldg(reinterpret_cast<const uint4*>(a)), hi = __ldg(reinterpret_cast<const uint4*>(a) + 1);
    e[0] = lo.x; e[1] = lo.y; e[2] = lo.z; e[3] = lo.w;
    e[4] = hi.x; e[5] = hi.y; e[6] = hi.z; e[7] = hi.w;
}
__device__ __forceinline__ bool eq32_aligned(const uint8_t* a, const uint32_t (&e)[8])
{
    uint32_t d[8];
    load32_aligned(a, d);
    uint32_t diff = 0;
#pragma unroll
    for (int i = 0; i < 8; ++i) diff |= d[i] ^ e[i];
    return diff == 0;
}
__device__ __forceinline__ void load32(const uint8_t* a, uint32_t (&e)[8])
{
    const uintptr_t p = (uintptr_t)a;
    const uint4* q = reinterpret_cast<const uint4*>(p & ~(uintptr_t)15);
    const uint4 q0 = __ldg(q), q1 = __ldg(q + 1), q2 = __ldg(q + 2);
    const uint32_t v[12] = {q0.x, q0.y, q0.z, q0.w, q1.x, q1.y, q1.z, q1.w, q2.x, q2.y, q2.z, q2.w};
    const uint32_t w0 = (uint32_t)(p & 15) >> 2, sh = (uint32_t)(p & 3) * 8;
    uint32_t u[9];
#pragma unroll
    for (int i = 0; i < 9; ++i) {
        const uint32_t a01 = (w0 & 1) ? v[i + 1] : v[i];
        const uint32_t a23 = (w0 & 1) ? v[i + 3 < 12 ? i + 3 : 11] : v[i + 2 < 12 ? i + 2 : 11];
        u[i] = (w0 & 2) ? a23 : a01;
    }
#pragma unroll
    for (int i = 0; i < 8; ++i) e[i] = __funnelshift_r(u[i], u[i + 1], sh);
}
__device__ __forceinline__ bool eq32_const(const uint8_t* a, const uint32_t (&e)[8])
{
    uint32_t diff = 0;
#pragma unroll
    for (int i = 0; i < 8; ++i) {
        const uint32_t w = (uint32_t)a[4 * i] | ((uint32_t)a[4 * i + 1] << 8) | ((uint32_t)a[4 * i + 2] << 16) | ((uint32_t)a[4 * i + 3] << 24);
        diff |= w ^ e[i];
    }
    return diff == 0;
}

__constant__ uint8_t EMPTY_ROOT[32] = {0x56, 0xe8, 0x1f, 0x17, 0x1b, 0xcc, 0x55, 0xa6, 0xff, 0x83, 0x45,
                                       0xe6, 0x92, 0xc0, 0xf8, 0x6e, 0x5b, 0x48, 0xe0, 0x1b, 0x99, 0x6c,
                                       0xad, 0xc0, 0x01, 0x62, 0x2f, 0xb5, 0xe3, 0x63, 0xb4, 0x21};

__device__ __forceinline__ uint32_t bag_slot(const uint32_t (&e)[8], uint32_t mask)
{
    uint64_t h = ((uint64_t)e[1] << 32) | e[0];
    h ^= h >> 29; h *= 0xBF58476D1CE4E5B9ull; h ^= h >> 32;
    return (uint32_t)h & mask;
}
__device__ uint32_t bag_find(const Bag& bag, const uint8_t* __restrict__ digests, const uint32_t (&expect)[8])
{
    uint32_t s = bag_slot(expect, bag.mask);
    for (;;) {
        const uint32_t idx = bag.table[s];
        if (idx == BAG_EMPTY) return BAG_EMPTY;
        if (eq32_aligned(digests + 32ull * idx, expect)) return idx;
        s = (s + 1) & bag.mask;
    }
}

template <bool BAG>
__device__ int walk_one(const uint8_t* __restrict__ nodes, const uint64_t* __restrict__ node_off,
                        const uint64_t* __restrict__ node_index, const Bag bag, uint64_t first,
                        uint64_t last, const uint8_t* __restrict__ key, const uint8_t* __restrict__ root,
                        const uint8_t* __restrict__ digests, const uint32_t* __restrict__ summary, uint64_t& voff, uint32_t& vlen)
{
    voff = 0; vlen = 0;
    uint32_t expect[8];
    load32_aligned(root, expect);
    uint32_t kw[8];
    load32_aligned(key, kw);
    auto key_nibble = [&](uint32_t q) -> uint32_t {
        const uint32_t wi = q >> 3;
        const uint32_t a01 = (wi & 1) ? kw[1] : kw[0], a23 = (wi & 1) ? kw[3] : kw[2], a45 = (wi & 1) ? kw[5] : kw[4], a67 = (wi & 1) ? kw[7] : kw[6];
        const uint32_t lo4 = (wi & 2) ? a23 : a01, hi4 = (wi & 2) ? a67 : a45;
        const uint32_t w = (wi & 4) ? hi4 : lo4;
        const uint32_t byte = (w >> (8 * ((q >> 1) & 3))) & 0xffu;
        return (q & 1) ? (byte & 15u) : (byte >> 4);
    };
    if (BAG) {
        first = 0;
        last = 1;
        if (eq32_const(EMPTY_ROOT, expect)) return ST_ABSENT;
    } else if (first == last) return eq32_const(EMPTY_ROOT, expect) ? ST_ABSENT : ST_REJECT;

    uint32_t pos = 0;
    uint64_t i = first;
    const uint8_t* cur = nullptr;
    uint32_t cur_len = 0;
    bool embedded = false;

    for (;;) {
        if (!embedded) {
            uint64_t ni;
            if (BAG) {
                const uint32_t f = bag_find(bag, digests, expect);
                if (f == BAG_EMPTY) return ST_MISSING;
                ni = f;
                i = last - 1;
            } else {
                if (i == last) return ST_REJECT;
                ni = node_index ? node_index[i] : i;
            }
            const uint64_t o = node_off[ni];
            const uint64_t l = node_off[ni + 1] - o;
            if (l > 0xffffffffull) return ST_REJECT;
            cur = nodes + o;
            cur_len = (uint32_t)l;
            if (!BAG && !eq32_aligned(digests + 32 * ni, expect)) return ST_REJECT;
            const uint32_t sm = summary ? summary[ni] : 0;
            ++i;
            if ((sm & 3u) == 1u && pos < 64) {
                const uint32_t nibble = key_nibble(pos);
                ++pos;
                const uint32_t mask = sm >> 8;
                if (!((mask >> nibble) & 1u)) return i == last ? ST_ABSENT : ST_REJECT;
                const uint32_t before = __popc(mask & ((1u << nibble) - 1u));
                load32(cur + ((sm >> 2) & 7u) + 33u * before + (nibble - before) + 1u, expect);
                continue;
            }
        }
        Item top;
        const uint32_t tot = rlp_item(cur, cur_len, top);
        if (tot == 0 || !top.is_list || tot != cur_len) return ST_REJECT;
        const uint8_t* pay = cur + top.pay_off;
        const uint32_t pl = top.pay_len;

        const uint32_t want = pos < 64 ? key_nibble(pos) : 16u;
        Item it0{}, it1{}, itw{}, it16{};
        uint32_t off0 = 0, off1 = 0, offw = 0, off16 = 0;
        uint32_t cnt = 0, o = 0;
        while (o < pl) {
            if (cnt == 17) return ST_REJECT;
            Item it;
            const uint32_t t = rlp_item(pay + o, pl - o, it);
            if (t == 0) return ST_REJECT;
            if (cnt == 0) { it0 = it; off0 = o; }
            if (cnt == 1) { it1 = it; off1 = o; }
            if (cnt == want) { itw = it; offw = o; }
            if (cnt == 16) { it16 = it; off16 = o; }
            o += t;
            ++cnt;
        }
        if (cnt != 17 && cnt != 2) return ST_REJECT;

        Item child;
        uint32_t child_off;
        if (cnt == 17) {
            if (pos == 64) {
                if (it16.is_list || i != last) return ST_REJECT;
                if (it16.pay_len == 0) return ST_ABSENT;
                voff = (uint64_t)(pay + off16 + it16.pay_off - nodes);
                vlen = it16.pay_len;
                return ST_PRESENT;
            }
            child = itw; child_off = offw;
            ++pos;
        } else {
            if (it0.is_list || it0.pay_len == 0) return ST_REJECT;
            const uint8_t* hp = pay + off0 + it0.pay_off;
            const uint32_t flag = hp[0] >> 4;
            if (flag > 3) return ST_REJECT;
            if (!(flag & 1) && (hp[0] & 15)) return ST_REJECT;
            const uint32_t plen = 2 * (it0.pay_len - 1) + (flag & 1);
            if (plen > 64) return ST_REJECT;
            bool match = 64 - pos >= plen;
            if ((flag & 2) && pos + plen != 64) match = false;
            else if (match && (flag & 2) && plen >= 2 && (uint64_t)(hp + it0.pay_len - nodes) >= 48) {
                uint32_t tail[8];
                load32(hp + it0.pay_len - 32, tail);
                const uint32_t nb = plen >> 1;
                uint32_t diff = 0;
#pragma unroll
                for (int w = 0; w < 8; ++w) {
                    const int first = 32 - (int)nb - 4 * w;
                    const uint32_t m = first <= 0 ? 0xffffffffu : (first >= 4 ? 0u : 0xffffffffu << (8 * first));
                    diff |= (tail[w] ^ kw[w]) & m;
                }
                if ((flag & 1) && (hp[0] & 15u) != key_nibble(pos)) diff = 1;
                match = diff == 0;
            } else if (match) {
                for (uint32_t j = 0; j < plen; ++j) {
                    const uint32_t q = j + 2 - (flag & 1);
                    const uint32_t pn = (q & 1) ? (hp[q >> 1] & 15u) : (hp[q >> 1] >> 4);
                    if (pn != key_nibble(pos + j)) { match = false; break; }
                }
            }
            if (flag & 2) {
                if (it1.is_list || i != last) return ST_REJECT;
                if (match && pos + plen == 64) {
                    voff = (uint64_t)(pay + off1 + it1.pay_off - nodes);
                    vlen = it1.pay_len;
                    return ST_PRESENT;
                }
                return ST_ABSENT;
            }
            if (plen == 0) return ST_REJECT;
            if (!match) return i == last ? ST_ABSENT : ST_REJECT;
            pos += plen;
            child = it1; child_off = off1;
        }
        if (child.is_list) {
            const uint32_t tot_child = child.pay_off + child.pay_len;
            if (tot_child >= 32) return ST_REJECT;
            cur = pay + child_off;
            cur_len = tot_child;
            embedded = true;
            continue;
        }
        embedded = false;
        if (child.pay_len == 0) {
            if (cnt == 2) return ST_REJECT;
            return i == last ? ST_ABSENT : ST_REJECT;
        }
        if (child.pay_len != 32) return ST_REJECT;
        load32(pay + child_off + child.pay_off, expect);
    }
}

}
}
```

Measured before the change: 132.5 million.

## Fuse Keccak hashing and MPT walk into a single per-proof verify kernel

Adds a fused verify kernel that hashes each proof's nodes and walks the trie in one pass. This removes the separate keccak launch and the round trip of digests and summaries through global memory. Classification and regrouping can now bin whole proofs by their total permutation count, and the walk logic is split into a per-node routine that works over an abstract byte source so it can read from shared memory. It also adds an aligned fast path for shared-memory absorbs, and falls back to the old path when the direct or warp keccak variants or node_index dedup are in use.

Result: faster. 137.0 million, median of 6 (+3.4%).

```diff
diff --git a/phant_b200/csrc/abi.cu b/phant_b200/csrc/abi.cu
--- a/phant_b200/csrc/abi.cu
+++ b/phant_b200/csrc/abi.cu
@@ -198,7 +198,7 @@
     if (int rc = d_perms.reserve(ctx, 64)) return rc;
     if (!perms_init) { CU(cudaMemsetAsync(d_perms.ptr, 0, 64, stream)); perms_init = true; }
     if (int rc = d_idx.reserve(ctx, keccak_regroup_scratch_bytes(device, n))) return rc;
-    CU(launch_keccak_classify(stream, device, d_off, n, (uint32_t*)d_idx.ptr, (uint32_t*)((unsigned long long*)d_perms.ptr + 1),
+    CU(launch_keccak_classify(stream, device, d_off, nullptr, n, (uint32_t*)d_idx.ptr, (uint32_t*)((unsigned long long*)d_perms.ptr + 1),
                               (unsigned long long*)d_perms.ptr));
     stats.launches++;
     perms_pending = true;
@@ -206,7 +206,7 @@
     const bool regroup = !(flags & PHANT_GPU_FLAG_NO_BINNING) && variant != KECCAK_WARP && n >= 4096;
     if (regroup) {
         if (int rc = d_order.reserve(ctx, 4 * n)) return rc;
-        CU(launch_keccak_regroup(stream, device, d_off, n, (const uint32_t*)d_idx.ptr, (uint32_t*)d_order.ptr));
+        CU(launch_keccak_regroup(stream, device, d_off, nullptr, n, (const uint32_t*)d_idx.ptr, (uint32_t*)d_order.ptr));
         stats.launches++;
         order = (const uint32_t*)d_order.ptr;
     }
@@ -279,6 +279,44 @@
     if (n == 0) return PHANT_GPU_OK;
     CU(cudaSetDevice(ctx->device));
     return ctx->hash_csr(msgs, off, n, total_bytes, out);
+}
+
+static bool fused_path(const phant_gpu_ctx* ctx, const uint8_t* nodes)
+{
+    return !(ctx->flags & (PHANT_GPU_FLAG_KECCAK_DIRECT | PHANT_GPU_FLAG_KECCAK_WARP)) && verify_fused_supported(nodes);
+}
+static int verify_fused(phant_gpu_ctx* ctx, const uint8_t* nodes, const uint64_t* node_off, const uint64_t* proof_first, uint64_t np,
+                        uint64_t n_nodes, uint64_t total, const uint8_t* keys32, const uint8_t* roots32, uint64_t n_roots, uint64_t* bitmap,
+                        uint8_t* status, uint64_t* val_off, uint32_t* val_len, const PeerOut* peer, bool fence_and_clear)
+{
+    if (np > 0xffffffffull) return PHANT_GPU_E_INVALID;
+    NvtxRange nvtx("phant:verify");
+    cudaStream_t s = ctx->stream;
+    if (int rc = ctx->d_perms.reserve(ctx, 64)) return rc;
+    if (!ctx->perms_init) { CU(cudaMemsetAsync(ctx->d_perms.ptr, 0, 64, s)); ctx->perms_init = true; }
+    const uint32_t* order = nullptr;
+    if (!peer && !(ctx->flags & PHANT_GPU_FLAG_NO_BINNING) && np >= 4096) {
+        if (int rc = ctx->d_idx.reserve(ctx, keccak_regroup_scratch_bytes(ctx->device, np))) return rc;
+        if (int rc = ctx->d_order.reserve(ctx, 4 * np)) return rc;
+        CU(launch_keccak_classify(s, ctx->device, node_off, proof_first, np, (uint32_t*)ctx->d_idx.ptr,
+                                  (uint32_t*)((unsigned long long*)ctx->d_perms.ptr + 1), nullptr));
+        CU(launch_keccak_regroup(s, ctx->device, node_off, proof_first, np, (const uint32_t*)ctx->d_idx.ptr, (uint32_t*)ctx->d_order.ptr));
+        ctx->stats.launches += 2;
+        order = (const uint32_t*)ctx->d_order.ptr;
+    }
+    if (fence_and_clear) {
+        if (int rc = ctx->wait_walk_fence()) return rc;
+        if (bitmap) CU(cudaMemsetAsync(bitmap, 0, ((np + 63) / 64) * 8, s));
+    }
+    ctx->time_begin(0);
+    CU(launch_verify_fused(s, ctx->device, np, nodes, node_off, proof_first, order, keys32, roots32, n_roots, bitmap, status, val_off, val_len,
+                           (unsigned long long*)ctx->d_perms.ptr, peer));
+    ctx->time_end();
+    ctx->stats.launches++;
+    ctx->stats.keccak_msgs += n_nodes;
+    ctx->stats.keccak_bytes += total;
+    ctx->perms_pending = true;
+    return PHANT_GPU_OK;
 }
 
 static int verify_dedup_host(phant_gpu_ctx* ctx, const phant_gpu_proof_batch* in, uint64_t* accept_bitmap, uint8_t* status,
@@ -355,6 +393,9 @@
                 CU(cudaStreamSynchronize(ctx->stream));
             }
         }
+        if (!in->node_index && fused_path(ctx, in->nodes))
+            return verify_fused(ctx, in->nodes, in->node_off, in->proof_first, np, n_nodes, total, in->keys32, in->roots32, in->n_roots,
+                                accept_bitmap, status, val_off, val_len, (const PeerOut*)ctx->walk_peer, true);
         if (int rc = ctx->d_digests.reserve(ctx, 32 * n_nodes + 32)) return rc;
         if (int rc = ctx->d_summary.reserve(ctx, 4 * n_nodes + 32)) return rc;
         if (int rc = ctx->hash_csr(in->nodes, in->node_off, n_nodes, total, (uint8_t*)ctx->d_digests.ptr, (uint32_t*)ctx->d_summary.ptr)) return rc;
@@ -379,8 +420,11 @@
     if (int rc = ctx->d_first.reserve(ctx, 8 * (np + 1))) return rc;
     if (int rc = ctx->d_keys.reserve(ctx, 32 * np)) return rc;
     if (int rc = ctx->d_roots.reserve(ctx, 32 * in->n_roots)) return rc;
-    if (int rc = ctx->d_digests.reserve(ctx, 32 * n_nodes + 32)) return rc;
-    if (int rc = ctx->d_summary.reserve(ctx, 4 * n_nodes + 32)) return rc;
+    const bool fused = fused_path(ctx, (const uint8_t*)ctx->d_msgs.ptr);
+    if (!fused) {
+        if (int rc = ctx->d_digests.reserve(ctx, 32 * n_nodes + 32)) return rc;
+        if (int rc = ctx->d_summary.reserve(ctx, 4 * n_nodes + 32)) return rc;
+    }
     if (int rc = ctx->d_bitmap.reserve(ctx, bm_bytes)) return rc;
     if (int rc = ctx->d_status.reserve(ctx, np)) return rc;
     if (val_off) if (int rc = ctx->d_voff.reserve(ctx, 8 * np)) return rc;
@@ -434,6 +478,19 @@
         CU(cudaEventRecord(ctx->chunk_events[chunk], cs));
         CU(cudaStreamWaitEvent(s, ctx->chunk_events[chunk], 0));
         nvtxRangePop();
+        if (fused) {
+            if (int rc = verify_fused(ctx, d_nodes, d_noff, d_pfirst + p0, p1 - p0, n1 - n0, b1 - b0, (const uint8_t*)ctx->d_keys.ptr + 32 * p0,
+                                      (const uint8_t*)ctx->d_roots.ptr + (in->n_roots == 1 ? 0 : 32 * p0), in->n_roots,
+                                      (uint64_t*)ctx->d_bitmap.ptr + p0 / 64, (uint8_t*)ctx->d_status.ptr + p0,
+                                      val_off ? (uint64_t*)ctx->d_voff.ptr + p0 : nullptr, val_len ? (uint32_t*)ctx->d_vlen.ptr + p0 : nullptr,
+                                      nullptr, false)) {
+                cudaStreamSynchronize(cs);
+                cudaStreamSynchronize(s);
+                return rc;
+            }
+            p0 = p1;
+            continue;
+        }
         if (int rc = ctx->hash_csr(d_nodes, d_noff + n0, n1 - n0, b1 - b0, (uint8_t*)ctx->d_digests.ptr + 32 * n0,
                                    (uint32_t*)ctx->d_summary.ptr + n0)) {
             cudaStreamSynchronize(cs);
diff --git a/phant_b200/csrc/common.cuh b/phant_b200/csrc/common.cuh
--- a/phant_b200/csrc/common.cuh
+++ b/phant_b200/csrc/common.cuh
@@ -11,9 +11,10 @@
                           const uint32_t* order, uint64_t n, uint8_t* out, uint32_t* summary ,
                           const uint64_t* len = nullptr );
 uint64_t keccak_regroup_scratch_bytes(int device, uint64_t n);
-cudaError_t launch_keccak_classify(cudaStream_t s, int device, const uint64_t* off, uint64_t n, uint32_t* hist, uint32_t* ticket,
-                                   unsigned long long* perms);
-cudaError_t launch_keccak_regroup(cudaStream_t s, int device, const uint64_t* off, uint64_t n, const uint32_t* start, uint32_t* order);
+cudaError_t launch_keccak_classify(cudaStream_t s, int device, const uint64_t* off, const uint64_t* first , uint64_t n,
+                                   uint32_t* hist, uint32_t* ticket, unsigned long long* perms );
+cudaError_t launch_keccak_regroup(cudaStream_t s, int device, const uint64_t* off, const uint64_t* first , uint64_t n,
+                                  const uint32_t* start, uint32_t* order);
 
 constexpr int PEER_MAX_WORLD = 16;
 struct PeerOut {
@@ -31,6 +32,12 @@
                         const uint64_t* node_index , const uint64_t* proof_first, const uint8_t* keys32, const uint8_t* roots32, uint64_t n_roots,
                         const uint8_t* digests, const uint32_t* summary , uint64_t* bitmap, uint8_t* status,
                         uint64_t* val_off, uint32_t* val_len, const PeerOut* peer = nullptr );
+
+bool verify_fused_supported(const uint8_t* nodes);
+cudaError_t launch_verify_fused(cudaStream_t s, int device, uint64_t n_proofs, const uint8_t* nodes, const uint64_t* node_off,
+                                const uint64_t* proof_first, const uint32_t* order, const uint8_t* keys32, const uint8_t* roots32,
+                                uint64_t n_roots, uint64_t* bitmap, uint8_t* status, uint64_t* val_off, uint32_t* val_len,
+                                unsigned long long* perms, const PeerOut* peer = nullptr);
 
 cudaError_t launch_peer_collect(cudaStream_t s, const unsigned long long* ready, uint32_t world, unsigned long long step, const void* src, void* dst,
                                 uint64_t bytes, const PeerOut& sig);
diff --git a/phant_b200/csrc/keccak_f1600.cuh b/phant_b200/csrc/keccak_f1600.cuh
--- a/phant_b200/csrc/keccak_f1600.cuh
+++ b/phant_b200/csrc/keccak_f1600.cuh
@@ -142,18 +142,23 @@
 __device__ __forceinline__ uint32_t lds32(uint32_t saddr) { uint32_t v; memcpy(&v, PHANT_HOST_SMEM + saddr, 4); return v; }
 #endif
 template <int UNROLL, bool DIGEST_ONLY = false>
-__device__ __forceinline__ void absorb_full_smem(uint64_t (&st)[25], uint32_t sa)
-{
-    const uint32_t a4 = sa & ~3u, sh = (sa & 3u) * 8;
-    uint32_t w[2 * KECCAK_RATE_WORDS + 1];
-#pragma unroll
-    for (int j = 0; j < 2 * KECCAK_RATE_WORDS; ++j) w[j] = lds32(a4 + 4 * j);
-    w[2 * KECCAK_RATE_WORDS] = sh ? lds32(a4 + 4 * 2 * KECCAK_RATE_WORDS) : 0;
-#pragma unroll
-    for (int k = 0; k < KECCAK_RATE_WORDS; ++k) {
-        const uint32_t lo = __funnelshift_r(w[2 * k], w[2 * k + 1], sh);
-        const uint32_t hi = __funnelshift_r(w[2 * k + 1], w[2 * k + 2], sh);
-        st[k] ^= ((uint64_t)hi << 32) | lo;
+__device__ __forceinline__ void absorb_full_smem(uint64_t (&st)[25], uint32_t sa, bool aligned = false)
+{
+    if (aligned) {
+#pragma unroll
+        for (int k = 0; k < KECCAK_RATE_WORDS; ++k) st[k] ^= ((uint64_t)lds32(sa + 8 * k + 4) << 32) | lds32(sa + 8 * k);
+    } else {
+        const uint32_t a4 = sa & ~3u, sh = (sa & 3u) * 8;
+        uint32_t w[2 * KECCAK_RATE_WORDS + 1];
+#pragma unroll
+        for (int j = 0; j < 2 * KECCAK_RATE_WORDS; ++j) w[j] = lds32(a4 + 4 * j);
+        w[2 * KECCAK_RATE_WORDS] = sh ? lds32(a4 + 4 * 2 * KECCAK_RATE_WORDS) : 0;
+#pragma unroll
+        for (int k = 0; k < KECCAK_RATE_WORDS; ++k) {
+            const uint32_t lo = __funnelshift_r(w[2 * k], w[2 * k + 1], sh);
+            const uint32_t hi = __funnelshift_r(w[2 * k + 1], w[2 * k + 2], sh);
+            st[k] ^= ((uint64_t)hi << 32) | lo;
+        }
     }
     keccak_f1600<UNROLL, DIGEST_ONLY>(st);
 }
@@ -184,7 +189,7 @@
     keccak_f1600<UNROLL, true>(st);
 }
 template <int UNROLL>
-__device__ __forceinline__ void absorb_final_smem(uint64_t (&st)[25], uint32_t sa, uint32_t rem, uint32_t room)
+__device__ __forceinline__ void absorb_final_smem(uint64_t (&st)[25], uint32_t sa, uint32_t rem, uint32_t room, bool aligned = false)
 {
     if (room < KECCAK_RATE + 4) { absorb_final_smem_masked<UNROLL>(st, sa, rem); return; }
     const uint32_t a4 = sa & ~3u, s = sa & 3u;
@@ -196,7 +201,7 @@
     sts32_(a4 + 4 * q0, w0);
     for (uint32_t q = q0 + 1; q < q1; ++q) sts32_(a4 + 4 * q, 0u);
     if (q1 > q0) sts32_(a4 + 4 * q1, 0x80u << (8 * b1));
-    absorb_full_smem<UNROLL, true>(st, sa);
+    absorb_full_smem<UNROLL, true>(st, sa, aligned);
 }
 
 template <int UNROLL = 2>
diff --git a/phant_b200/csrc/keccak_kernels.cu b/phant_b200/csrc/keccak_kernels.cu
--- a/phant_b200/csrc/keccak_kernels.cu
+++ b/phant_b200/csrc/keccak_kernels.cu
@@ -1,6 +1,7 @@
 #include "common.cuh"
 #include "keccak_f1600.cuh"
 #include "node_summary.cuh"
+#include "stage.cuh"
 
 #include <stdlib.h>
 #include <string.h>
@@ -23,48 +24,6 @@
         o[0] = dg[0]; o[1] = dg[1]; o[2] = dg[2]; o[3] = dg[3];
     }
 }
-
-constexpr int stage_window(int blocks)
-{
-    int s = (blocks * KECCAK_RATE + 15 + 15) / 16;
-    if (s % 2 == 0) ++s;
-    return 16 * s;
-}
-constexpr int stage_slot(int blocks) { return stage_window(blocks) + 32; }
-constexpr int stage_smem(int blocks, int warps) { return 128 + warps * 32 * stage_slot(blocks) + 16; }
-static_assert(stage_smem(4, 12) <= 232448, "default shape must fit the 227 KB a CTA may opt into");
-
-__device__ __forceinline__ uint32_t smem_u32(const void* p) { return (uint32_t)__cvta_generic_to_shared(p); }
-__device__ __forceinline__ void mbar_init(uint32_t bar, uint32_t count)
-{
-    asm volatile("mbarrier.init.shared::cta.b64 [%0], %1;" ::"r"(bar), "r"(count));
-}
-__device__ __forceinline__ void mbar_arrive(uint32_t bar)
-{
-    asm volatile("mbarrier.arrive.shared::cta.b64 _, [%0];" ::"r"(bar) : "memory");
-}
-__device__ __forceinline__ void mbar_arrive_expect_tx(uint32_t bar, uint32_t bytes)
-{
-    asm volatile("mbarrier.arrive.expect_tx.shared::cta.b64 _, [%0], %1;" ::"r"(bar), "r"(bytes) : "memory");
-}
-__device__ __forceinline__ void mbar_wait(uint32_t bar, uint32_t parity)
-{
-    asm volatile(
-        "{\n"
-        ".reg .pred P1;\n"
-        "LAB_WAIT:\n"
-        "mbarrier.try_wait.parity.shared::cta.b64 P1, [%0], %1;\n"
-        "@P1 bra DONE;\n"
-        "bra LAB_WAIT;\n"
-        "DONE:\n"
-        "}" ::"r"(bar), "r"(parity) : "memory");
-}
-__device__ __forceinline__ void bulk_g2s(uint32_t dst, const void* src, uint32_t bytes, uint32_t bar)
-{
-    asm volatile("cp.async.bulk.shared::cluster.global.mbarrier::complete_tx::bytes [%0], [%1], %2, [%3];"
-                 ::"r"(dst), "l"(src), "r"(bytes), "r"(bar) : "memory");
-}
-__device__ __forceinline__ void fence_proxy_async() { asm volatile("fence.proxy.async.shared::cta;" ::: "memory"); }
 
 template <int UNROLL, int BLOCKS, int WARPS>
 __global__ void __launch_bounds__(WARPS * 32)
@@ -114,6 +73,7 @@
             }
             mbar_wait(bar, parity);
             parity ^= 1;
+            const bool aligned = __all_sync(0xffffffffu, done || (cur & 3) == 0);
             if (!done) {
                 const uint32_t skew = (uint32_t)(cur - a0);
                 const uint64_t in_slot = cs - skew;
@@ -123,11 +83,11 @@
                 const uint32_t nfull = (uint32_t)(avail / KECCAK_RATE);
                 uint32_t sa = slot_s + skew;
                 for (uint32_t b = 0; b < nfull; ++b) {
-                    absorb_full_smem<UNROLL>(st, sa);
+                    absorb_full_smem<UNROLL>(st, sa, aligned);
                     sa += KECCAK_RATE;
                 }
                 if (avail == need) {
-                    absorb_final_smem<UNROLL>(st, sa, (uint32_t)(avail - (uint64_t)nfull * KECCAK_RATE), slot_s + SLOT - sa);
+                    absorb_final_smem<UNROLL>(st, sa, (uint32_t)(avail - (uint64_t)nfull * KECCAK_RATE), slot_s + SLOT - sa, aligned);
                     done = true;
                 } else {
                     cur += (uint64_t)nfull * KECCAK_RATE;
@@ -217,15 +177,22 @@
 
 constexpr int CLS_THREADS = 256, CLS_WARPS = CLS_THREADS / 32;
 
-__device__ __forceinline__ uint32_t keccak_class_of(uint64_t len)
-{
-    const uint64_t nb = len / KECCAK_RATE + 1;
-    return (uint32_t)(15 - (nb > 16 ? 15 : nb - 1));
+__device__ __forceinline__ uint64_t keccak_item_perms(const uint64_t* __restrict__ off, const uint64_t* __restrict__ first, uint64_t i)
+{
+    if (!first) return (off[i + 1] - off[i]) / KECCAK_RATE + 1;
+    uint64_t nb = 0;
+    for (uint64_t j = first[i], e = first[i + 1]; j < e; ++j) nb += (off[j + 1] - off[j]) / KECCAK_RATE + 1;
+    return nb;
+}
+__device__ __forceinline__ uint32_t keccak_class_of(uint64_t nb, bool proofs)
+{
+    const uint64_t c = proofs ? (nb ? (nb - 1) / 4 : 0) : nb - 1;
+    return (uint32_t)(15 - (c > 15 ? 15 : c));
 }
 
 __global__ void __launch_bounds__(CLS_THREADS)
-keccak_class_kernel(const uint64_t* __restrict__ off, uint64_t n, uint64_t chunk, uint32_t* __restrict__ hist ,
-                    uint32_t* __restrict__ ticket, unsigned long long* __restrict__ perms)
+keccak_class_kernel(const uint64_t* __restrict__ off, const uint64_t* __restrict__ first, uint64_t n, uint64_t chunk,
+                    uint32_t* __restrict__ hist , uint32_t* __restrict__ ticket, unsigned long long* __restrict__ perms)
 {
     __shared__ uint32_t h[16];
     __shared__ uint32_t cls_total[16];
@@ -239,15 +206,15 @@
         const bool valid = i < hi;
         uint32_t c = 16;
         if (valid) {
-            const uint64_t len = off[i + 1] - off[i];
-            c = keccak_class_of(len);
-            local += len / KECCAK_RATE + 1;
+            const uint64_t nb = keccak_item_perms(off, first, i);
+            c = keccak_class_of(nb, first != nullptr);
+            local += nb;
         }
         const uint32_t peers = __match_any_sync(0xffffffffu, c);
         if (valid && (threadIdx.x & 31) == (uint32_t)(__ffs(peers) - 1)) atomicAdd(&h[c], __popc(peers));
     }
     for (int o = 16; o; o >>= 1) local += __shfl_down_sync(0xffffffffu, local, o);
-    if ((threadIdx.x & 31) == 0 && local) atomicAdd(perms, local);
+    if ((threadIdx.x & 31) == 0 && local && perms) atomicAdd(perms, local);
     __syncthreads();
     if (threadIdx.x < 16) hist[16 * blockIdx.x + threadIdx.x] = h[threadIdx.x];
     __threadfence();
@@ -283,8 +250,8 @@
 }
 
 __global__ void __launch_bounds__(CLS_THREADS)
-keccak_regroup_kernel(const uint64_t* __restrict__ off, uint64_t n, uint64_t chunk, const uint32_t* __restrict__ start ,
-                      uint32_t* __restrict__ order)
+keccak_regroup_kernel(const uint64_t* __restrict__ off, const uint64_t* __restrict__ first, uint64_t n, uint64_t chunk,
+                      const uint32_t* __restrict__ start , uint32_t* __restrict__ order)
 {
     __shared__ uint32_t base[16];
     __shared__ uint32_t wcnt[CLS_WARPS][16];
@@ -296,7 +263,7 @@
         __syncthreads();
         const uint64_t i = i0 + threadIdx.x;
         const bool valid = i < hi;
-        const uint32_t c = valid ? keccak_class_of(off[i + 1] - off[i]) : 16;
+        const uint32_t c = valid ? keccak_class_of(keccak_item_perms(off, first, i), first != nullptr) : 16;
         const uint32_t peers = __match_any_sync(0xffffffffu, c);
         const uint32_t rank = __popc(peers & ((1u << lane) - 1u));
         if (valid && rank == 0) wcnt[warp][c] = __popc(peers);
@@ -408,21 +375,22 @@
     class_geometry(device, n ? n : 1, blocks, chunk);
     return 64 * blocks;
 }
-cudaError_t launch_keccak_classify(cudaStream_t s, int device, const uint64_t* off, uint64_t n, uint32_t* hist, uint32_t* ticket,
-                                   unsigned long long* perms)
+cudaError_t launch_keccak_classify(cudaStream_t s, int device, const uint64_t* off, const uint64_t* first, uint64_t n, uint32_t* hist,
+                                   uint32_t* ticket, unsigned long long* perms)
 {
     if (n == 0) return cudaSuccess;
     uint64_t blocks, chunk;
     class_geometry(device, n, blocks, chunk);
-    keccak_class_kernel<<<(unsigned)blocks, CLS_THREADS, 0, s>>>(off, n, chunk, hist, ticket, perms);
+    keccak_class_kernel<<<(unsigned)blocks, CLS_THREADS, 0, s>>>(off, first, n, chunk, hist, ticket, perms);
     return cudaGetLastError();
 }
-cudaError_t launch_keccak_regroup(cudaStream_t s, int device, const uint64_t* off, uint64_t n, const uint32_t* start, uint32_t* order)
+cudaError_t launch_keccak_regroup(cudaStream_t s, int device, const uint64_t* off, const uint64_t* first, uint64_t n, const uint32_t* start,
+                                  uint32_t* order)
 {
     if (n == 0) return cudaSuccess;
     uint64_t blocks, chunk;
     class_geometry(device, n, blocks, chunk);
-    keccak_regroup_kernel<<<(unsigned)blocks, CLS_THREADS, 0, s>>>(off, n, chunk, start, order);
+    keccak_regroup_kernel<<<(unsigned)blocks, CLS_THREADS, 0, s>>>(off, first, n, chunk, start, order);
     return cudaGetLastError();
 }
 
diff --git a/phant_b200/csrc/peer_sync.cuh b/phant_b200/csrc/peer_sync.cuh
--- /dev/null
+++ b/phant_b200/csrc/peer_sync.cuh
@@ -0,0 +1,32 @@
+#pragma once
+#include <stdint.h>
+
+namespace phant {
+namespace {
+
+__device__ __forceinline__ unsigned long long ld_acquire_sys(const unsigned long long* p)
+{
+    unsigned long long v;
+    asm volatile("ld.acquire.sys.global.u64 %0, [%1];" : "=l"(v) : "l"(p) : "memory");
+    return v;
+}
+__device__ __forceinline__ void st_release_sys(unsigned long long* p, unsigned long long v)
+{
+    asm volatile("st.release.sys.global.u64 [%0], %1;" ::"l"(p), "l"(v) : "memory");
+}
+__device__ __forceinline__ unsigned long long global_timer_ns()
+{
+    unsigned long long t;
+    asm volatile("mov.u64 %0, %globaltimer;" : "=l"(t));
+    return t;
+}
+__device__ __forceinline__ void wait_flags(const unsigned long long* flags, uint32_t world, unsigned long long value, uint32_t* err)
+{
+    const unsigned long long t0 = global_timer_ns();
+    for (uint32_t r = 0; r < world; ++r)
+        while (ld_acquire_sys(flags + r) < value)
+            if (global_timer_ns() - t0 > 4000000000ull) { *err = 1; return; }
+}
+
+}
+}
diff --git a/phant_b200/csrc/stage.cuh b/phant_b200/csrc/stage.cuh
--- /dev/null
+++ b/phant_b200/csrc/stage.cuh
@@ -0,0 +1,50 @@
+#pragma once
+#include <stdint.h>
+
+#include "keccak_f1600.cuh"
+
+namespace phant {
+
+constexpr int stage_window(int blocks)
+{
+    int s = (blocks * KECCAK_RATE + 15 + 15) / 16;
+    if (s % 2 == 0) ++s;
+    return 16 * s;
+}
+constexpr int stage_slot(int blocks) { return stage_window(blocks) + 32; }
+constexpr int stage_smem(int blocks, int warps) { return 128 + warps * 32 * stage_slot(blocks) + 16; }
+static_assert(stage_smem(4, 12) <= 232448, "default shape must fit the 227 KB a CTA may opt into");
+
+__device__ __forceinline__ uint32_t smem_u32(const void* p) { return (uint32_t)__cvta_generic_to_shared(p); }
+__device__ __forceinline__ void mbar_init(uint32_t bar, uint32_t count)
+{
+    asm volatile("mbarrier.init.shared::cta.b64 [%0], %1;" ::"r"(bar), "r"(count));
+}
+__device__ __forceinline__ void mbar_arrive(uint32_t bar)
+{
+    asm volatile("mbarrier.arrive.shared::cta.b64 _, [%0];" ::"r"(bar) : "memory");
+}
+__device__ __forceinline__ void mbar_arrive_expect_tx(uint32_t bar, uint32_t bytes)
+{
+    asm volatile("mbarrier.arrive.expect_tx.shared::cta.b64 _, [%0], %1;" ::"r"(bar), "r"(bytes) : "memory");
+}
+__device__ __forceinline__ void mbar_wait(uint32_t bar, uint32_t parity)
+{
+    asm volatile(
+        "{\n"
+        ".reg .pred P1;\n"
+        "LAB_WAIT:\n"
+        "mbarrier.try_wait.parity.shared::cta.b64 P1, [%0], %1;\n"
+        "@P1 bra DONE;\n"
+        "bra LAB_WAIT;\n"
+        "DONE:\n"
+        "}" ::"r"(bar), "r"(parity) : "memory");
+}
+__device__ __forceinline__ void bulk_g2s(uint32_t dst, const void* src, uint32_t bytes, uint32_t bar)
+{
+    asm volatile("cp.async.bulk.shared::cluster.global.mbarrier::complete_tx::bytes [%0], [%1], %2, [%3];"
+                 ::"r"(dst), "l"(src), "r"(bytes), "r"(bar) : "memory");
+}
+__device__ __forceinline__ void fence_proxy_async() { asm volatile("fence.proxy.async.shared::cta;" ::: "memory"); }
+
+}
diff --git a/phant_b200/csrc/verify_fused.cu b/phant_b200/csrc/verify_fused.cu
--- /dev/null
+++ b/phant_b200/csrc/verify_fused.cu
@@ -0,0 +1,204 @@
+#include "common.cuh"
+#include "keccak_f1600.cuh"
+#include "node_summary.cuh"
+#include "peer_sync.cuh"
+#include "stage.cuh"
+#include "walk_one.cuh"
+
+namespace phant {
+namespace {
+
+template <int UNROLL, int BLOCKS, int WARPS, bool PEER>
+__global__ void __launch_bounds__(WARPS * 32, 1)
+verify_fused_kernel(uint64_t n_proofs, const uint8_t* __restrict__ nodes, const uint64_t* __restrict__ node_off,
+                    const uint64_t* __restrict__ proof_first, const uint32_t* __restrict__ order, const uint8_t* __restrict__ keys32,
+                    const uint8_t* __restrict__ roots32, uint64_t n_roots, uint64_t* __restrict__ bitmap, uint8_t* __restrict__ status,
+                    uint64_t* __restrict__ val_off, uint32_t* __restrict__ val_len, unsigned long long* __restrict__ perms, const PeerOut peer)
+{
+    extern __shared__ __align__(128) uint8_t smem[];
+    const uint32_t warp = threadIdx.x >> 5, lane = threadIdx.x & 31;
+    const uint32_t bar = smem_u32(smem) + 8 * warp;
+    constexpr int SLOT = stage_slot(BLOCKS), WINDOW = stage_window(BLOCKS);
+    uint8_t* slot = smem + 128 + (warp * 32 + lane) * SLOT;
+    const uint32_t slot_s = smem_u32(slot);
+    if (lane == 0) mbar_init(bar, 32);
+    fence_proxy_async();
+    if (PEER) {
+        if (threadIdx.x == 0 && peer.wait_done) wait_flags(peer.done, peer.world, peer.wait_done, peer.err);
+    }
+    __syncthreads();
+    uint32_t parity = 0;
+    uint64_t my_perms = 0;
+
+    const uint64_t n_tiles = (n_proofs + 31) / 32;
+    for (uint64_t tile = (uint64_t)blockIdx.x * WARPS + warp; tile < n_tiles; tile += (uint64_t)gridDim.x * WARPS) {
+        const uint64_t idx = tile * 32 + lane;
+        const bool active = idx < n_proofs;
+        uint64_t p = 0, j = 0, jl = 0, nbeg = 0, cur = 0, end = 0, nxt = 0, voff = 0;
+        uint32_t vlen = 0, pos = 0;
+        uint32_t expect[8], kw[8];
+        int verdict = ST_REJECT;
+        bool done = !active;
+        if (active) {
+            p = order ? order[idx] : idx;
+            j = proof_first[p];
+            jl = proof_first[p + 1];
+            load32_aligned(roots32 + (n_roots == 1 ? 0 : 32 * p), expect);
+            load32_aligned(keys32 + 32 * p, kw);
+            if (j == jl) {
+                verdict = eq32_const(EMPTY_ROOT, expect) ? ST_ABSENT : ST_REJECT;
+                done = true;
+            } else {
+                nbeg = cur = node_off[j];
+                end = node_off[j + 1];
+                if (j + 1 < jl) nxt = node_off[j + 2];
+                if (end - nbeg > 0xffffffffull) done = true;
+            }
+        }
+        uint64_t st[25];
+#pragma unroll
+        for (int i = 0; i < 25; ++i) st[i] = 0;
+        bool first_trip = true;
+
+        while (!__all_sync(0xffffffffu, done)) {
+            const uint64_t need = done ? 0 : end - cur;
+            const uint64_t a0 = cur & ~(uint64_t)15;
+            uint32_t cs = 0;
+            if (need) {
+                const uint64_t span = ((end - a0) + 15) & ~(uint64_t)15;
+                cs = span < WINDOW ? (uint32_t)span : WINDOW;
+                fence_proxy_async();
+                mbar_arrive_expect_tx(bar, cs);
+                bulk_g2s(slot_s, nodes + a0, cs, bar);
+            } else {
+                mbar_arrive(bar);
+            }
+            mbar_wait(bar, parity);
+            parity ^= 1;
+            const bool aligned = __all_sync(0xffffffffu, done || (cur & 3) == 0);
+            if (done) continue;
+            const uint32_t skew = (uint32_t)(cur - a0);
+            const uint64_t in_slot = cs - skew;
+            const uint64_t avail = need < in_slot ? need : in_slot;
+            const uint32_t nfull = (uint32_t)(avail / KECCAK_RATE);
+            uint32_t sa = slot_s + skew;
+            for (uint32_t b = 0; b < nfull; ++b) {
+                absorb_full_smem<UNROLL>(st, sa, aligned);
+                sa += KECCAK_RATE;
+            }
+            my_perms += nfull;
+            if (avail != need) {
+                cur += (uint64_t)nfull * KECCAK_RATE;
+                first_trip = false;
+                continue;
+            }
+            absorb_final_smem<UNROLL>(st, sa, (uint32_t)(avail - (uint64_t)nfull * KECCAK_RATE), slot_s + SLOT - sa, aligned);
+            ++my_perms;
+            uint32_t diff = 0;
+#pragma unroll
+            for (int w = 0; w < 4; ++w) diff |= ((uint32_t)st[w] ^ expect[2 * w]) | ((uint32_t)(st[w] >> 32) ^ expect[2 * w + 1]);
+            const uint32_t len = (uint32_t)(end - nbeg);
+            int r = ST_REJECT;
+            ++j;
+            if (diff == 0) {
+                if (first_trip) {
+                    const uint8_t* np = slot + skew;
+                    r = walk_node(SlotBytes{np, skew, nbeg}, len, summarize_node(np, len), j == jl, kw, pos, expect, voff, vlen);
+                } else {
+                    r = walk_node(GlobalBytes{nodes, nbeg}, len, 0u, j == jl, kw, pos, expect, voff, vlen);
+                }
+                if (r == ST_NEXT && j == jl) r = ST_REJECT;
+            }
+            if (r != ST_NEXT) {
+                verdict = r;
+                done = true;
+                continue;
+            }
+            nbeg = cur = end;
+            end = nxt;
+            if (j + 1 < jl) nxt = node_off[j + 2];
+            if (end - nbeg > 0xffffffffull) { done = true; continue; }
+#pragma unroll
+            for (int i = 0; i < 25; ++i) st[i] = 0;
+            first_trip = true;
+        }
+
+        if (active) {
+            if (status) status[p] = (uint8_t)verdict;
+            if (val_off) val_off[p] = verdict == ST_PRESENT ? voff : 0;
+            if (val_len) val_len[p] = verdict == ST_PRESENT ? vlen : 0;
+        }
+        const bool acc = active && (verdict == ST_PRESENT || verdict == ST_ABSENT);
+        const uint32_t word = __ballot_sync(0xffffffffu, acc);
+        if (PEER) {
+            if (lane < peer.world) peer.dst[lane][tile] = word;
+        } else if (bitmap) {
+            if (__all_sync(0xffffffffu, !active || p == idx)) {
+                if (lane == 0) reinterpret_cast<uint32_t*>(bitmap)[tile] = word;
+            } else if (acc) {
+                atomicOr(reinterpret_cast<uint32_t*>(bitmap) + (p >> 5), 1u << (p & 31));
+            }
+        }
+    }
+    for (int o = 16; o; o >>= 1) my_perms += __shfl_down_sync(0xffffffffu, my_perms, o);
+    if (lane == 0 && my_perms) atomicAdd(perms, (unsigned long long)my_perms);
+    if (PEER) {
+        __threadfence_system();
+        __syncthreads();
+        if (threadIdx.x == 0) {
+            const uint32_t t = atomicAdd(peer.ticket, 1u);
+            if (t == gridDim.x - 1) {
+                __threadfence_system();
+                for (uint32_t r = 0; r < peer.world; ++r) st_release_sys(peer.ready[r], peer.step);
+                *peer.ticket = 0;
+            }
+        }
+    }
+}
+
+template <bool PEER>
+cudaError_t launch_fused(cudaStream_t s, int device, uint64_t n_proofs, const uint8_t* nodes, const uint64_t* node_off,
+                         const uint64_t* proof_first, const uint32_t* order, const uint8_t* keys32, const uint8_t* roots32, uint64_t n_roots,
+                         uint64_t* bitmap, uint8_t* status, uint64_t* val_off, uint32_t* val_len, unsigned long long* perms, const PeerOut& peer)
+{
+    constexpr int BLOCKS = 4, WARPS = 12;
+    constexpr int SMEM = stage_smem(BLOCKS, WARPS);
+    auto kernel = verify_fused_kernel<2, BLOCKS, WARPS, PEER>;
+    static int ctas_cache[64] = {0};
+    int& ctas_per_sm = ctas_cache[(device >= 0 && device < 64) ? device : 0];
+    if (!ctas_per_sm) {
+        cudaError_t e = cudaFuncSetAttribute(kernel, cudaFuncAttributeMaxDynamicSharedMemorySize, SMEM);
+        if (e != cudaSuccess) return e;
+        cudaFuncSetAttribute(kernel, cudaFuncAttributePreferredSharedMemoryCarveout, 100);
+        e = cudaOccupancyMaxActiveBlocksPerMultiprocessor(&ctas_per_sm, kernel, WARPS * 32, SMEM);
+        if (e != cudaSuccess || ctas_per_sm < 1) { ctas_per_sm = 0; return e != cudaSuccess ? e : cudaErrorLaunchOutOfResources; }
+    }
+    const uint64_t tiles = (n_proofs + 31) / 32;
+    uint64_t blocks = (tiles + WARPS - 1) / WARPS;
+    const uint64_t cap = (uint64_t)keccak_num_sms(device) * ctas_per_sm;
+    if (blocks > cap) blocks = cap;
+    kernel<<<(unsigned)blocks, WARPS * 32, SMEM, s>>>(n_proofs, nodes, node_off, proof_first, order, keys32, roots32, n_roots, bitmap, status,
+                                                      val_off, val_len, perms, peer);
+    return cudaGetLastError();
+}
+
+}
+
+bool verify_fused_supported(const uint8_t* nodes) { return ((uintptr_t)nodes & 15) == 0; }
+
+cudaError_t launch_verify_fused(cudaStream_t s, int device, uint64_t n_proofs, const uint8_t* nodes, const uint64_t* node_off,
+                                const uint64_t* proof_first, const uint32_t* order, const uint8_t* keys32, const uint8_t* roots32,
+                                uint64_t n_roots, uint64_t* bitmap, uint8_t* status, uint64_t* val_off, uint32_t* val_len,
+                                unsigned long long* perms, const PeerOut* peer)
+{
+    if (n_proofs == 0) return cudaSuccess;
+    if (peer) {
+        if (order) return cudaErrorInvalidValue;
+        return launch_fused<true>(s, device, n_proofs, nodes, node_off, proof_first, nullptr, keys32, roots32, n_roots, bitmap, status, val_off,
+                                  val_len, perms, *peer);
+    }
+    return launch_fused<false>(s, device, n_proofs, nodes, node_off, proof_first, order, keys32, roots32, n_roots, bitmap, status, val_off,
+                               val_len, perms, PeerOut{});
+}
+
+}
diff --git a/phant_b200/csrc/walk_kernel.cu b/phant_b200/csrc/walk_kernel.cu
--- a/phant_b200/csrc/walk_kernel.cu
+++ b/phant_b200/csrc/walk_kernel.cu
@@ -2,34 +2,11 @@
 
 #include <stdlib.h>
 
+#include "peer_sync.cuh"
 #include "walk_one.cuh"
 
 namespace phant {
 namespace {
-
-__device__ __forceinline__ unsigned long long ld_acquire_sys(const unsigned long long* p)
-{
-    unsigned long long v;
-    asm volatile("ld.acquire.sys.global.u64 %0, [%1];" : "=l"(v) : "l"(p) : "memory");
-    return v;
-}
-__device__ __forceinline__ void st_release_sys(unsigned long long* p, unsigned long long v)
-{
-    asm volatile("st.release.sys.global.u64 [%0], %1;" ::"l"(p), "l"(v) : "memory");
-}
-__device__ __forceinline__ unsigned long long global_timer_ns()
-{
-    unsigned long long t;
-    asm volatile("mov.u64 %0, %globaltimer;" : "=l"(t));
-    return t;
-}
-__device__ __forceinline__ void wait_flags(const unsigned long long* flags, uint32_t world, unsigned long long value, uint32_t* err)
-{
-    const unsigned long long t0 = global_timer_ns();
-    for (uint32_t r = 0; r < world; ++r)
-        while (ld_acquire_sys(flags + r) < value)
-            if (global_timer_ns() - t0 > 4000000000ull) { *err = 1; return; }
-}
 
 template <bool BAG, int MINB, bool PEER = false>
 __global__ void __launch_bounds__(128, MINB)
diff --git a/phant_b200/csrc/walk_one.cuh b/phant_b200/csrc/walk_one.cuh
--- a/phant_b200/csrc/walk_one.cuh
+++ b/phant_b200/csrc/walk_one.cuh
@@ -18,10 +18,106 @@
     uint32_t pay_len;
 };
 
-__device__ __forceinline__ uint32_t rlp_item(const uint8_t* p, uint32_t avail, Item& it)
+__device__ __forceinline__ void load32_aligned(const uint8_t* a, uint32_t (&e)[8])
+{
+    const uint4 lo = __ldg(reinterpret_cast<const uint4*>(a)), hi = __ldg(reinterpret_cast<const uint4*>(a) + 1);
+    e[0] = lo.x; e[1] = lo.y; e[2] = lo.z; e[3] = lo.w;
+    e[4] = hi.x; e[5] = hi.y; e[6] = hi.z; e[7] = hi.w;
+}
+__device__ __forceinline__ bool eq32_aligned(const uint8_t* a, const uint32_t (&e)[8])
+{
+    uint32_t d[8];
+    load32_aligned(a, d);
+    uint32_t diff = 0;
+#pragma unroll
+    for (int i = 0; i < 8; ++i) diff |= d[i] ^ e[i];
+    return diff == 0;
+}
+__device__ __forceinline__ void load32(const uint8_t* a, uint32_t (&e)[8])
+{
+    const uintptr_t p = (uintptr_t)a;
+    const uint4* q = reinterpret_cast<const uint4*>(p & ~(uintptr_t)15);
+    const uint4 q0 = __ldg(q), q1 = __ldg(q + 1), q2 = __ldg(q + 2);
+    const uint32_t v[12] = {q0.x, q0.y, q0.z, q0.w, q1.x, q1.y, q1.z, q1.w, q2.x, q2.y, q2.z, q2.w};
+    const uint32_t w0 = (uint32_t)(p & 15) >> 2, sh = (uint32_t)(p & 3) * 8;
+    uint32_t u[9];
+#pragma unroll
+    for (int i = 0; i < 9; ++i) {
+        const uint32_t a01 = (w0 & 1) ? v[i + 1] : v[i];
+        const uint32_t a23 = (w0 & 1) ? v[i + 3 < 12 ? i + 3 : 11] : v[i + 2 < 12 ? i + 2 : 11];
+        u[i] = (w0 & 2) ? a23 : a01;
+    }
+#pragma unroll
+    for (int i = 0; i < 8; ++i) e[i] = __funnelshift_r(u[i], u[i + 1], sh);
+}
+__device__ __forceinline__ bool eq32_const(const uint8_t* a, const uint32_t (&e)[8])
+{
+    uint32_t diff = 0;
+#pragma unroll
+    for (int i = 0; i < 8; ++i) {
+        const uint32_t w = (uint32_t)a[4 * i] | ((uint32_t)a[4 * i + 1] << 8) | ((uint32_t)a[4 * i + 2] << 16) | ((uint32_t)a[4 * i + 3] << 24);
+        diff |= w ^ e[i];
+    }
+    return diff == 0;
+}
+
+__constant__ uint8_t EMPTY_ROOT[32] = {0x56, 0xe8, 0x1f, 0x17, 0x1b, 0xcc, 0x55, 0xa6, 0xff, 0x83, 0x45,
+                                       0xe6, 0x92, 0xc0, 0xf8, 0x6e, 0x5b, 0x48, 0xe0, 0x1b, 0x99, 0x6c,
+                                       0xad, 0xc0, 0x01, 0x62, 0x2f, 0xb5, 0xe3, 0x63, 0xb4, 0x21};
+
+__device__ __forceinline__ uint32_t bag_slot(const uint32_t (&e)[8], uint32_t mask)
+{
+    uint64_t h = ((uint64_t)e[1] << 32) | e[0];
+    h ^= h >> 29; h *= 0xBF58476D1CE4E5B9ull; h ^= h >> 32;
+    return (uint32_t)h & mask;
+}
+__device__ uint32_t bag_find(const Bag& bag, const uint8_t* __restrict__ digests, const uint32_t (&expect)[8])
+{
+    uint32_t s = bag_slot(expect, bag.mask);
+    for (;;) {
+        const uint32_t idx = bag.table[s];
+        if (idx == BAG_EMPTY) return BAG_EMPTY;
+        if (eq32_aligned(digests + 32ull * idx, expect)) return idx;
+        s = (s + 1) & bag.mask;
+    }
+}
+
+struct GlobalBytes {
+    const uint8_t* __restrict__ nodes;
+    uint64_t base;
+    __device__ __forceinline__ uint32_t at(uint32_t o) const { return nodes[base + o]; }
+    __device__ __forceinline__ void load32(uint32_t o, uint32_t (&e)[8]) const { ::phant::load32(nodes + base + o, e); }
+    __device__ __forceinline__ bool tail_ok(uint32_t e) const { return base + e >= 48; }
+    __device__ __forceinline__ void load32_tail(uint32_t e, uint32_t (&t)[8]) const { ::phant::load32(nodes + (base + e - 32), t); }
+    __device__ __forceinline__ uint64_t abs(uint32_t o) const { return base + o; }
+};
+struct SlotBytes {
+    const uint8_t* p;
+    uint32_t skew;
+    uint64_t base;
+    __device__ __forceinline__ uint32_t at(uint32_t o) const { return p[o]; }
+    __device__ __forceinline__ void load32(uint32_t o, uint32_t (&e)[8]) const { load32_at(p + o, e); }
+    __device__ __forceinline__ void load32_tail(uint32_t e, uint32_t (&t)[8]) const { load32_at(p + e - 32, t); }
+    __device__ __forceinline__ static void load32_at(const uint8_t* q, uint32_t (&e)[8])
+    {
+        const uintptr_t a = (uintptr_t)q;
+        const uint32_t* w = reinterpret_cast<const uint32_t*>(a & ~(uintptr_t)3);
+        const uint32_t sh = (uint32_t)(a & 3) * 8;
+        uint32_t u[9];
+#pragma unroll
+        for (int i = 0; i < 9; ++i) u[i] = w[i];
+#pragma unroll
+        for (int i = 0; i < 8; ++i) e[i] = __funnelshift_r(u[i], u[i + 1], sh);
+    }
+    __device__ __forceinline__ bool tail_ok(uint32_t e) const { return skew + e >= 32; }
+    __device__ __forceinline__ uint64_t abs(uint32_t o) const { return base + o; }
+};
+
+template <class Bytes>
+__device__ __forceinline__ uint32_t rlp_item_at(const Bytes& nb, uint32_t at, uint32_t avail, Item& it)
 {
     if (avail == 0) return 0;
-    const uint32_t b = p[0];
+    const uint32_t b = nb.at(at);
     if (b < 0x80) { it.is_list = 0; it.pay_off = 0; it.pay_len = 1; return 1; }
     const uint32_t is_list = b >= 0xc0;
     const uint32_t base_short = is_list ? 0xc0 : 0x80, base_long = is_list ? 0xf7 : 0xb7;
@@ -29,160 +125,61 @@
     if (b <= base_long) {
         const uint32_t len = b - base_short;
         if (1 + len > avail) return 0;
-        if (!is_list && len == 1 && p[1] < 0x80) return 0;
+        if (!is_list && len == 1 && nb.at(at + 1) < 0x80) return 0;
         it.pay_off = 1; it.pay_len = len;
         return 1 + len;
     }
     const uint32_t n = b - base_long;
     if (n > 4 || 1 + n > avail) return 0;
-    if (p[1] == 0) return 0;
+    if (nb.at(at + 1) == 0) return 0;
     uint64_t len = 0;
-    for (uint32_t i = 0; i < n; ++i) len = (len << 8) | p[1 + i];
+    for (uint32_t i = 0; i < n; ++i) len = (len << 8) | nb.at(at + 1 + i);
     if (len <= 55) return 0;
     if (1 + n + len > avail) return 0;
     it.pay_off = 1 + n; it.pay_len = (uint32_t)len;
     return (uint32_t)(1 + n + len);
 }
 
-__device__ __forceinline__ void load32_aligned(const uint8_t* a, uint32_t (&e)[8])
-{
-    const uint4 lo = __ldg(reinterpret_cast<const uint4*>(a)), hi = __ldg(reinterpret_cast<const uint4*>(a) + 1);
-    e[0] = lo.x; e[1] = lo.y; e[2] = lo.z; e[3] = lo.w;
-    e[4] = hi.x; e[5] = hi.y; e[6] = hi.z; e[7] = hi.w;
-}
-__device__ __forceinline__ bool eq32_aligned(const uint8_t* a, const uint32_t (&e)[8])
-{
-    uint32_t d[8];
-    load32_aligned(a, d);
-    uint32_t diff = 0;
-#pragma unroll
-    for (int i = 0; i < 8; ++i) diff |= d[i] ^ e[i];
-    return diff == 0;
-}
-__device__ __forceinline__ void load32(const uint8_t* a, uint32_t (&e)[8])
-{
-    const uintptr_t p = (uintptr_t)a;
-    const uint4* q = reinterpret_cast<const uint4*>(p & ~(uintptr_t)15);
-    const uint4 q0 = __ldg(q), q1 = __ldg(q + 1), q2 = __ldg(q + 2);
-    const uint32_t v[12] = {q0.x, q0.y, q0.z, q0.w, q1.x, q1.y, q1.z, q1.w, q2.x, q2.y, q2.z, q2.w};
-    const uint32_t w0 = (uint32_t)(p & 15) >> 2, sh = (uint32_t)(p & 3) * 8;
-    uint32_t u[9];
-#pragma unroll
-    for (int i = 0; i < 9; ++i) {
-        const uint32_t a01 = (w0 & 1) ? v[i + 1] : v[i];
-        const uint32_t a23 = (w0 & 1) ? v[i + 3 < 12 ? i + 3 : 11] : v[i + 2 < 12 ? i + 2 : 11];
-        u[i] = (w0 & 2) ? a23 : a01;
-    }
-#pragma unroll
-    for (int i = 0; i < 8; ++i) e[i] = __funnelshift_r(u[i], u[i + 1], sh);
-}
-__device__ __forceinline__ bool eq32_const(const uint8_t* a, const uint32_t (&e)[8])
-{
-    uint32_t diff = 0;
-#pragma unroll
-    for (int i = 0; i < 8; ++i) {
-        const uint32_t w = (uint32_t)a[4 * i] | ((uint32_t)a[4 * i + 1] << 8) | ((uint32_t)a[4 * i + 2] << 16) | ((uint32_t)a[4 * i + 3] << 24);
-        diff |= w ^ e[i];
-    }
-    return diff == 0;
-}
-
-__constant__ uint8_t EMPTY_ROOT[32] = {0x56, 0xe8, 0x1f, 0x17, 0x1b, 0xcc, 0x55, 0xa6, 0xff, 0x83, 0x45,
-                                       0xe6, 0x92, 0xc0, 0xf8, 0x6e, 0x5b, 0x48, 0xe0, 0x1b, 0x99, 0x6c,
-                                       0xad, 0xc0, 0x01, 0x62, 0x2f, 0xb5, 0xe3, 0x63, 0xb4, 0x21};
-
-__device__ __forceinline__ uint32_t bag_slot(const uint32_t (&e)[8], uint32_t mask)
-{
-    uint64_t h = ((uint64_t)e[1] << 32) | e[0];
-    h ^= h >> 29; h *= 0xBF58476D1CE4E5B9ull; h ^= h >> 32;
-    return (uint32_t)h & mask;
-}
-__device__ uint32_t bag_find(const Bag& bag, const uint8_t* __restrict__ digests, const uint32_t (&expect)[8])
-{
-    uint32_t s = bag_slot(expect, bag.mask);
+__device__ __forceinline__ uint32_t key_nibble(const uint32_t (&kw)[8], uint32_t q)
+{
+    const uint32_t wi = q >> 3;
+    const uint32_t a01 = (wi & 1) ? kw[1] : kw[0], a23 = (wi & 1) ? kw[3] : kw[2], a45 = (wi & 1) ? kw[5] : kw[4], a67 = (wi & 1) ? kw[7] : kw[6];
+    const uint32_t lo4 = (wi & 2) ? a23 : a01, hi4 = (wi & 2) ? a67 : a45;
+    const uint32_t w = (wi & 4) ? hi4 : lo4;
+    const uint32_t byte = (w >> (8 * ((q >> 1) & 3))) & 0xffu;
+    return (q & 1) ? (byte & 15u) : (byte >> 4);
+}
+
+enum { ST_NEXT = 4 };
+template <class Bytes>
+__device__ __forceinline__ int walk_node(const Bytes& nb, uint32_t len, uint32_t sm, bool last_node, const uint32_t (&kw)[8], uint32_t& pos,
+                                         uint32_t (&expect)[8], uint64_t& voff, uint32_t& vlen)
+{
+    if ((sm & 3u) == 1u && pos < 64) {
+        const uint32_t nibble = key_nibble(kw, pos);
+        ++pos;
+        const uint32_t mask = sm >> 8;
+        if (!((mask >> nibble) & 1u)) return last_node ? ST_ABSENT : ST_REJECT;
+        const uint32_t before = __popc(mask & ((1u << nibble) - 1u));
+        nb.load32(((sm >> 2) & 7u) + 33u * before + (nibble - before) + 1u, expect);
+        return ST_NEXT;
+    }
+    uint32_t cur = 0, cur_len = len;
     for (;;) {
-        const uint32_t idx = bag.table[s];
-        if (idx == BAG_EMPTY) return BAG_EMPTY;
-        if (eq32_aligned(digests + 32ull * idx, expect)) return idx;
-        s = (s + 1) & bag.mask;
-    }
-}
-
-template <bool BAG>
-__device__ int walk_one(const uint8_t* __restrict__ nodes, const uint64_t* __restrict__ node_off,
-                        const uint64_t* __restrict__ node_index, const Bag bag, uint64_t first,
-                        uint64_t last, const uint8_t* __restrict__ key, const uint8_t* __restrict__ root,
-                        const uint8_t* __restrict__ digests, const uint32_t* __restrict__ summary, uint64_t& voff, uint32_t& vlen)
-{
-    voff = 0; vlen = 0;
-    uint32_t expect[8];
-    load32_aligned(root, expect);
-    uint32_t kw[8];
-    load32_aligned(key, kw);
-    auto key_nibble = [&](uint32_t q) -> uint32_t {
-        const uint32_t wi = q >> 3;
-        const uint32_t a01 = (wi & 1) ? kw[1] : kw[0], a23 = (wi & 1) ? kw[3] : kw[2], a45 = (wi & 1) ? kw[5] : kw[4], a67 = (wi & 1) ? kw[7] : kw[6];
-        const uint32_t lo4 = (wi & 2) ? a23 : a01, hi4 = (wi & 2) ? a67 : a45;
-        const uint32_t w = (wi & 4) ? hi4 : lo4;
-        const uint32_t byte = (w >> (8 * ((q >> 1) & 3))) & 0xffu;
-        return (q & 1) ? (byte & 15u) : (byte >> 4);
-    };
-    if (BAG) {
-        first = 0;
-        last = 1;
-        if (eq32_const(EMPTY_ROOT, expect)) return ST_ABSENT;
-    } else if (first == last) return eq32_const(EMPTY_ROOT, expect) ? ST_ABSENT : ST_REJECT;
-
-    uint32_t pos = 0;
-    uint64_t i = first;
-    const uint8_t* cur = nullptr;
-    uint32_t cur_len = 0;
-    bool embedded = false;
-
-    for (;;) {
-        if (!embedded) {
-            uint64_t ni;
-            if (BAG) {
-                const uint32_t f = bag_find(bag, digests, expect);
-                if (f == BAG_EMPTY) return ST_MISSING;
-                ni = f;
-                i = last - 1;
-            } else {
-                if (i == last) return ST_REJECT;
-                ni = node_index ? node_index[i] : i;
-            }
-            const uint64_t o = node_off[ni];
-            const uint64_t l = node_off[ni + 1] - o;
-            if (l > 0xffffffffull) return ST_REJECT;
-            cur = nodes + o;
-            cur_len = (uint32_t)l;
-            if (!BAG && !eq32_aligned(digests + 32 * ni, expect)) return ST_REJECT;
-            const uint32_t sm = summary ? summary[ni] : 0;
-            ++i;
-            if ((sm & 3u) == 1u && pos < 64) {
-                const uint32_t nibble = key_nibble(pos);
-                ++pos;
-                const uint32_t mask = sm >> 8;
-                if (!((mask >> nibble) & 1u)) return i == last ? ST_ABSENT : ST_REJECT;
-                const uint32_t before = __popc(mask & ((1u << nibble) - 1u));
-                load32(cur + ((sm >> 2) & 7u) + 33u * before + (nibble - before) + 1u, expect);
-                continue;
-            }
-        }
         Item top;
-        const uint32_t tot = rlp_item(cur, cur_len, top);
+        const uint32_t tot = rlp_item_at(nb, cur, cur_len, top);
         if (tot == 0 || !top.is_list || tot != cur_len) return ST_REJECT;
-        const uint8_t* pay = cur + top.pay_off;
+        const uint32_t pay = cur + top.pay_off;
         const uint32_t pl = top.pay_len;
 
-        const uint32_t want = pos < 64 ? key_nibble(pos) : 16u;
+        const uint32_t want = pos < 64 ? key_nibble(kw, pos) : 16u;
         Item it0{}, it1{}, itw{}, it16{};
         uint32_t off0 = 0, off1 = 0, offw = 0, off16 = 0;
         uint32_t cnt = 0, o = 0;
         while (o < pl) {
             if (cnt == 17) return ST_REJECT;
             Item it;
-            const uint32_t t = rlp_item(pay + o, pl - o, it);
+            const uint32_t t = rlp_item_at(nb, pay + o, pl - o, it);
             if (t == 0) return ST_REJECT;
             if (cnt == 0) { it0 = it; off0 = o; }
             if (cnt == 1) { it1 = it; off1 = o; }
@@ -197,9 +194,9 @@
         uint32_t child_off;
         if (cnt == 17) {
             if (pos == 64) {
-                if (it16.is_list || i != last) return ST_REJECT;
+                if (it16.is_list || !last_node) return ST_REJECT;
                 if (it16.pay_len == 0) return ST_ABSENT;
-                voff = (uint64_t)(pay + off16 + it16.pay_off - nodes);
+                voff = nb.abs(pay + off16 + it16.pay_off);
                 vlen = it16.pay_len;
                 return ST_PRESENT;
             }
@@ -207,45 +204,47 @@
             ++pos;
         } else {
             if (it0.is_list || it0.pay_len == 0) return ST_REJECT;
-            const uint8_t* hp = pay + off0 + it0.pay_off;
-            const uint32_t flag = hp[0] >> 4;
+            const uint32_t hp = pay + off0 + it0.pay_off;
+            const uint32_t h0 = nb.at(hp);
+            const uint32_t flag = h0 >> 4;
             if (flag > 3) return ST_REJECT;
-            if (!(flag & 1) && (hp[0] & 15)) return ST_REJECT;
+            if (!(flag & 1) && (h0 & 15)) return ST_REJECT;
             const uint32_t plen = 2 * (it0.pay_len - 1) + (flag & 1);
             if (plen > 64) return ST_REJECT;
             bool match = 64 - pos >= plen;
             if ((flag & 2) && pos + plen != 64) match = false;
-            else if (match && (flag & 2) && plen >= 2 && (uint64_t)(hp + it0.pay_len - nodes) >= 48) {
+            else if (match && (flag & 2) && plen >= 2 && nb.tail_ok(hp + it0.pay_len)) {
                 uint32_t tail[8];
-                load32(hp + it0.pay_len - 32, tail);
-                const uint32_t nb = plen >> 1;
+                nb.load32_tail(hp + it0.pay_len, tail);
+                const uint32_t nbytes = plen >> 1;
                 uint32_t diff = 0;
 #pragma unroll
                 for (int w = 0; w < 8; ++w) {
-                    const int first = 32 - (int)nb - 4 * w;
+                    const int first = 32 - (int)nbytes - 4 * w;
                     const uint32_t m = first <= 0 ? 0xffffffffu : (first >= 4 ? 0u : 0xffffffffu << (8 * first));
                     diff |= (tail[w] ^ kw[w]) & m;
                 }
-                if ((flag & 1) && (hp[0] & 15u) != key_nibble(pos)) diff = 1;
+                if ((flag & 1) && (h0 & 15u) != key_nibble(kw, pos)) diff = 1;
                 match = diff == 0;
             } else if (match) {
                 for (uint32_t j = 0; j < plen; ++j) {
                     const uint32_t q = j + 2 - (flag & 1);
-                    const uint32_t pn = (q & 1) ? (hp[q >> 1] & 15u) : (hp[q >> 1] >> 4);
-                    if (pn != key_nibble(pos + j)) { match = false; break; }
+                    const uint32_t hb = nb.at(hp + (q >> 1));
+                    const uint32_t pn = (q & 1) ? (hb & 15u) : (hb >> 4);
+                    if (pn != key_nibble(kw, pos + j)) { match = false; break; }
                 }
             }
             if (flag & 2) {
-                if (it1.is_list || i != last) return ST_REJECT;
+                if (it1.is_list || !last_node) return ST_REJECT;
                 if (match && pos + plen == 64) {
-                    voff = (uint64_t)(pay + off1 + it1.pay_off - nodes);
+                    voff = nb.abs(pay + off1 + it1.pay_off);
                     vlen = it1.pay_len;
                     return ST_PRESENT;
                 }
                 return ST_ABSENT;
             }
             if (plen == 0) return ST_REJECT;
-            if (!match) return i == last ? ST_ABSENT : ST_REJECT;
+            if (!match) return last_node ? ST_ABSENT : ST_REJECT;
             pos += plen;
             child = it1; child_off = off1;
         }
@@ -254,18 +253,58 @@
             if (tot_child >= 32) return ST_REJECT;
             cur = pay + child_off;
             cur_len = tot_child;
-            embedded = true;
             continue;
         }
-        embedded = false;
         if (child.pay_len == 0) {
             if (cnt == 2) return ST_REJECT;
-            return i == last ? ST_ABSENT : ST_REJECT;
+            return last_node ? ST_ABSENT : ST_REJECT;
         }
         if (child.pay_len != 32) return ST_REJECT;
-        load32(pay + child_off + child.pay_off, expect);
-    }
-}
-
-}
-}
+        nb.load32(pay + child_off + child.pay_off, expect);
+        return ST_NEXT;
+    }
+}
+
+template <bool BAG>
+__device__ int walk_one(const uint8_t* __restrict__ nodes, const uint64_t* __restrict__ node_off,
+                        const uint64_t* __restrict__ node_index, const Bag bag, uint64_t first,
+                        uint64_t last, const uint8_t* __restrict__ key, const uint8_t* __restrict__ root,
+                        const uint8_t* __restrict__ digests, const uint32_t* __restrict__ summary, uint64_t& voff, uint32_t& vlen)
+{
+    voff = 0; vlen = 0;
+    uint32_t expect[8];
+    load32_aligned(root, expect);
+    uint32_t kw[8];
+    load32_aligned(key, kw);
+    if (BAG) {
+        first = 0;
+        last = 1;
+        if (eq32_const(EMPTY_ROOT, expect)) return ST_ABSENT;
+    } else if (first == last) return eq32_const(EMPTY_ROOT, expect) ? ST_ABSENT : ST_REJECT;
+
+    uint32_t pos = 0;
+    uint64_t i = first;
+    for (;;) {
+        uint64_t ni;
+        if (BAG) {
+            const uint32_t f = bag_find(bag, digests, expect);
+            if (f == BAG_EMPTY) return ST_MISSING;
+            ni = f;
+            i = last - 1;
+        } else {
+            if (i == last) return ST_REJECT;
+            ni = node_index ? node_index[i] : i;
+        }
+        const uint64_t o = node_off[ni];
+        const uint64_t l = node_off[ni + 1] - o;
+        if (l > 0xffffffffull) return ST_REJECT;
+        if (!BAG && !eq32_aligned(digests + 32 * ni, expect)) return ST_REJECT;
+        const uint32_t sm = summary ? summary[ni] : 0;
+        ++i;
+        const int st = walk_node(GlobalBytes{nodes, o}, (uint32_t)l, sm, i == last, kw, pos, expect, voff, vlen);
+        if (st != ST_NEXT) return st;
+    }
+}
+
+}
+}
```
